# RishWijewardhena/vision-textile-inspection

Measured on AMD Instinct MI355X. Metric: frames/sec whole-node, YOLOv8n-seg 640x640 bs=64; mask IoU vs CPU ref, higher is better.
Workload: dtype f16x2

## Files before the change

vision-textile-inspection_amd/csrc/conv.hip:

```cpp
#include <algorithm>
#include <cstdlib>
#include <type_traits>

#include "conv_dev.h"

namespace vti {

__host__ __device__ inline int patch_dim(int t, int ks, int s, int mode) { return mode == 1 ? t : (t - 1) * s + ks; }

size_t stem_lds_bytes(int TH, int TW);

size_t conv_lds_bytes(int ks, int stride, int mode, int TH, int TW, int WN, int NREP) {
    if (mode == 1) return stem_lds_bytes(TH, TW);
    const int npix = patch_dim(TH, ks, stride, mode) * patch_dim(TW, ks, stride, mode);
    const size_t plane = (size_t)((npix + 15) & ~15) * 16;
    const int taps = mode == 1 ? 1 : ks * ks;
    size_t raw = 0;
    if (mode == 1) raw = (((size_t)(2 * TH + 1) * (2 * TW + 1) * 3) + 15) & ~(size_t)15;
    return 4 * plane + (size_t)WN * NREP * taps * 1024 + raw;
}

template <typename T, int KS, int S, int NREP, int WN, int NREP2 = 0, int NT = 256>
__global__ __launch_bounds__(NT, NT == 512 ? 1 : 2) void conv_kernel(const ConvParams p) {
    using vec = typename Tr<T>::vec;
    constexpr int VEC = Tr<T>::VEC, KC = Tr<T>::KC;
    constexpr int TAPS = KS * KS, PAD = KS / 2;
    constexpr int NTB = WN * NREP;
    constexpr int PP = NT / 4;
    constexpr int AR = NT == 512 ? 6 : (S == 2 ? 12 : 8);
    constexpr int BR = (NTB * TAPS * 64 + NT - 1) / NT;
    constexpr unsigned OOB = 0xFFFFFFFFu;
    extern __shared__ __attribute__((aligned(16))) char smem[];

    const int tid = threadIdx.x, lane = tid & 63, wave = tid >> 6;
    const int wn = wave % WN, wm = wave / WN;
    int t = blockIdx.x;
    const int tx = t % p.tiles_x; t /= p.tiles_x;
    const int ty = t % p.tiles_y;
    const int b = t / p.tiles_y;
    const int oy0 = ty * p.TH, ox0 = tx * p.TW;
    const int PH = (p.TH - 1) * S + KS, PW = (p.TW - 1) * S + KS;
    const int npix = PH * PW;
    const int plane_bytes = ((npix + 15) & ~15) * 16;
    char* smA = smem;
    char* smB = smem + 4 * plane_bytes;
    const int nt0 = blockIdx.y * NTB;
    const int tile_px = p.TH * p.TW;
    VTI_STAMP(0);

    int abase[MREP], opy[MREP], opx[MREP];
    bool pvalid[MREP];
#pragma unroll
    for (int m = 0; m < MREP; ++m) {
        const int pp = (wm * MREP + m) * 16 + (lane & 15);
        const bool v = pp < tile_px;
        const int pc = v ? pp : 0;
        const int py = (int)__umulhi((unsigned)pc, p.tw_magic), px = pc - py * p.TW;
        opy[m] = oy0 + py; opx[m] = ox0 + px;
        pvalid[m] = v && opy[m] < p.Hout && opx[m] < p.Wout;
        abase[m] = (lane >> 4) * plane_bytes + ((py * S) * PW + px * S) * 16;
    }

    f32x4 acc[MREP][NREP];
#pragma unroll
    for (int m = 0; m < MREP; ++m)
#pragma unroll
        for (int n = 0; n < NREP; ++n) acc[m][n] = (f32x4){0.f, 0.f, 0.f, 0.f};

    const size_t frame_elems = (size_t)p.Hin * p.Win * p.in_ld;
    const __amdgpu_buffer_rsrc_t rsA = __builtin_amdgcn_make_buffer_rsrc(
        (void*)((const T*)p.in + (size_t)b * frame_elems), 0, (int)(frame_elems * sizeof(T)), 0x00020000);
    const __amdgpu_buffer_rsrc_t rsB = __builtin_amdgcn_make_buffer_rsrc((void*)p.wpk, 0, (int)p.wpk_bytes, 0x00020000);

    const int iy0 = oy0 * S - PAD, ix0 = ox0 * S - PAD;
    const int q = (tid >> 3) & 3;
    const int pix0 = (tid >> 5) * 8 + (tid & 7);
    const int ldsA0 = q * plane_bytes + pix0 * 16;
    const int cvalid = (p.Cin - q * VEC + KC - 1) / KC;
    unsigned aoff[AR];
#pragma unroll
    for (int u = 0; u < AR; ++u) {
        const int pix = pix0 + PP * u;
        const int py = (int)__umulhi((unsigned)pix, p.pw_magic), px = pix - py * PW;
        const int y = iy0 + py, x = ix0 + px;
        const bool ok = pix < npix && (unsigned)y < (unsigned)p.Hin && (unsigned)x < (unsigned)p.Win;
        aoff[u] = ok ? (unsigned)(((y * p.Win + x) * p.in_ld + p.in_coff + q * VEC) * (int)sizeof(T)) : OOB;
    }
    constexpr bool BPRE = NREP < 5 || NT == 512;
    constexpr int PD = (KS == 1 && BPRE) ? 2 : 1;
    vec ra[PD][AR], rb[PD][BR];
    auto loadB = [&](int c, vec (&rbs)[BR]) {
        const unsigned sB = (unsigned)(((size_t)c * p.ntiles_n + nt0) * (TAPS * 1024));
#pragma unroll
        for (int u = 0; u < BR; ++u)
            if (tid + u * NT < NTB * TAPS * 64) rbs[u] = buf_load16<vec>(rsB, (unsigned)(tid + u * NT) * 16u, sB);
    };
    auto issue = [&](int c, vec (&ras)[AR], vec (&rbs)[BR]) {
        const bool qok = c < cvalid;
#pragma unroll
        for (int u = 0; u < AR; ++u)
            if (pix0 + PP * u < ((npix + 7) & ~7))
                ras[u] = buf_load16<vec>(rsA, qok ? aoff[u] : OOB, (unsigned)(c * KC * (int)sizeof(T)));
        if constexpr (BPRE) loadB(c, rbs);
    };
    auto commit = [&](int c, vec (&ras)[AR], vec (&rbs)[BR]) {
        if constexpr (!BPRE) loadB(c, rbs);
#pragma unroll
        for (int u = 0; u < AR; ++u)
            if (pix0 + PP * u < npix) *(vec*)(smA + ldsA0 + u * (PP * 16)) = ras[u];
#pragma unroll
        for (int u = 0; u < BR; ++u)
            if (tid + u * NT < NTB * TAPS * 64) *(vec*)(smB + (tid + u * NT) * 16) = rbs[u];
    };
    auto chunk = [&](int c, auto set_c) {
        constexpr int SET = decltype(set_c)::value;
        if (c < 2) VTI_STAMP(1 + 5 * c);
        commit(c, ra[SET], rb[SET]);
        if (c < 2) VTI_STAMP(3 + 5 * c);
        __syncthreads();
        if (c < 2) VTI_STAMP(4 + 5 * c);
        if (c + PD < p.nchunks) issue(c + PD, ra[SET], rb[SET]);
        {
            constexpr int NSTEP = TAPS * MREP;
            constexpr int XD = NREP >= 5 ? 2 : 3;
            constexpr int WD = NREP >= 5 ? 1 : 2;
            vec xq[XD];
            vec wq[WD][NREP];
            auto ldx = [&](int s_) -> vec {
                const int tp = s_ / MREP, mm = s_ % MREP;
                const int toff = ((tp / KS) * PW + (tp % KS)) * 16;
                return *(const vec*)(smA + abase[mm] + toff);
            };
            auto ldw = [&](int tp, vec (&w)[NREP]) {
#pragma unroll
                for (int n = 0; n < NREP; ++n)
                    w[n] = *(const vec*)(smB + ((wn * NREP + n) * TAPS + tp) * 1024 + lane * 16);
            };
            if constexpr (Tr<T>::H2 && TAPS > 1 && (NREP <= 3 || (NREP == 4 && NT == 512))) {
                auto ldw1 = [&](int tp, int n) -> vec { return *(const vec*)(smB + ((wn * NREP + n) * TAPS + tp) * 1024 + lane * 16); };
                h2_taps<NREP, MREP, TAPS, 3>(acc, ldx, ldw1);
            } else {
            ldw(0, wq[0]);
            xq[0] = ldx(0);
            if (XD > 2 && NSTEP > 1) xq[1] = ldx(1);
#pragma unroll
            for (int s_ = 0; s_ < NSTEP; ++s_) {
                const int tp = s_ / MREP, mm = s_ % MREP;
                if (s_ + XD - 1 < NSTEP) xq[(s_ + XD - 1) % XD] = ldx(s_ + XD - 1);
                if (WD == 2 && mm == 0 && tp + 1 < TAPS) ldw(tp + 1, wq[(tp + 1) % WD]);
                __builtin_amdgcn_sched_barrier(0);
#pragma unroll
                for (int n = 0; n < NREP; ++n) acc[mm][n] = mma(wq[tp % WD][n], xq[s_ % XD], acc[mm][n]);
                __builtin_amdgcn_sched_barrier(0);
                if (WD == 1 && mm == MREP - 1 && tp + 1 < TAPS) ldw(tp + 1, wq[0]);
            }
            }
        }
        if (c < 2) VTI_STAMP(5 + 5 * c);
        if (c + 1 < p.nchunks) __syncthreads();
    };

    issue(0, ra[0], rb[0]);
    if constexpr (PD == 2) {
        if (p.nchunks > 1) issue(1, ra[1], rb[1]);
        for (int c = 0; c < p.nchunks; c += 2) {
            chunk(c, std::integral_constant<int, 0>{});
            if (c + 1 < p.nchunks) chunk(c + 1, std::integral_constant<int, 1>{});
        }
    } else {
        for (int c = 0; c < p.nchunks; ++c) chunk(c, std::integral_constant<int, 0>{});
    }

    VTI_STAMP(11);
    if constexpr (NREP2 == 0) {
        conv_epilogue<T, NREP>(p, acc, pvalid, opy, opx, b, nt0, wn, lane);
    } else {
        static_assert(WN == 1, "fused stage needs the whole Cout in one wave");
        conv_stage2<T, NREP, NREP2>(p, acc, pvalid, opy, opx, b, lane);
    }
    VTI_STAMP(12);
}

size_t convfold_lds_bytes(int TH, int TW) {
    const int npix = (TH + 2) * (TW + 2);
    return 4 * (size_t)((npix + 15) & ~15) * 16 + (size_t)16 * 4 * 1024;
}
bool convfold_supported(int c_in, int c_mid, int c_out, int ntiles2) {
    return c_in == c_mid && c_mid % 16 == 0 && c_out == 64 && c_in % 16 == 0 && c_in <= 64 && combo_has(FoldN2{}, ntiles2);
}

template <typename T, int NREP2, int NT = 256>
__global__ __launch_bounds__(NT, NT == 512 ? 1 : 2) void convfold_kernel(const ConvParams p) {
    using vec = typename Tr<T>::vec;
    constexpr int VEC = Tr<T>::VEC, KC = Tr<T>::KC;
    constexpr int NREP = 4, TAPS = 4, NTB = 16, AR = 8;
    constexpr int BR = NTB * TAPS * 64 / NT;
    constexpr int PPP = NT / 4;
    constexpr unsigned OOB = 0xFFFFFFFFu;
    extern __shared__ __attribute__((aligned(16))) char smem[];

    const int tid = threadIdx.x, lane = tid & 63, wave = (tid >> 6) & 3, mgrp = tid >> 8;
    const int py = wave >> 1, px = wave & 1;
    int t = blockIdx.x;
    const int tx = t % p.tiles_x; t /= p.tiles_x;
    const int ty = t % p.tiles_y;
    const int b = t / p.tiles_y;
    const int oy0 = ty * p.TH, ox0 = tx * p.TW;
    const int PH = p.TH + 2, PW = p.TW + 2;
    const int npix = PH * PW;
    const int plane_bytes = ((npix + 15) & ~15) * 16;
    char* smA = smem;
    char* smB = smem + 4 * plane_bytes;
    const int tile_px = p.TH * p.TW;

    int abase[MREP], opy[MREP], opx[MREP];
    bool pvalid[MREP];
#pragma unroll
    for (int m = 0; m < MREP; ++m) {
        const int pp = (mgrp * MREP + m) * 16 + (lane & 15);
        const bool v = pp < tile_px;
        const int pc = v ? pp : 0;
        const int ly = (int)__umulhi((unsigned)pc, p.tw_magic), lx = pc - ly * p.TW;
        pvalid[m] = v && oy0 + ly < p.Hout && ox0 + lx < p.Wout;
        opy[m] = 2 * (oy0 + ly) + py; opx[m] = 2 * (ox0 + lx) + px;
        abase[m] = (lane >> 4) * plane_bytes + ((ly + py) * PW + lx + px) * 16;
    }
    f32x4 acc[MREP][NREP];
#pragma unroll
    for (int m = 0; m < MREP; ++m)
#pragma unroll
        for (int n = 0; n < NREP; ++n) acc[m][n] = (f32x4){0.f, 0.f, 0.f, 0.f};

    const size_t frame_elems = (size_t)p.Hin * p.Win * p.in_ld;
    const __amdgpu_buffer_rsrc_t rsA = __builtin_amdgcn_make_buffer_rsrc(
        (void*)((const T*)p.in + (size_t)b * frame_elems), 0, (int)(frame_elems * sizeof(T)), 0x00020000);
    const __amdgpu_buffer_rsrc_t rsB = __builtin_amdgcn_make_buffer_rsrc((void*)p.wpk, 0, (int)p.wpk_bytes, 0x00020000);
    const int iy0 = oy0 - 1, ix0 = ox0 - 1;
    const int q = (tid >> 3) & 3;
    const int pix0 = (tid >> 5) * 8 + (tid & 7);
    const int ldsA0 = q * plane_bytes + pix0 * 16;
    const int cvalid = (p.Cin - q * VEC + KC - 1) / KC;
    unsigned aoff[AR];
#pragma unroll
    for (int u = 0; u < AR; ++u) {
        const int pix = pix0 + PPP * u;
        const int ry = (int)__umulhi((unsigned)pix, p.pw_magic), rx = pix - ry * PW;
        const int y = iy0 + ry, x = ix0 + rx;
        const bool ok = pix < npix && (unsigned)y < (unsigned)p.Hin && (unsigned)x < (unsigned)p.Win;
        aoff[u] = ok ? (unsigned)(((y * p.Win + x) * p.in_ld + p.in_coff + q * VEC) * (int)sizeof(T)) : OOB;
    }
    vec ra[AR];
    auto issue = [&](int c) {
        const bool qok = c < cvalid;
#pragma unroll
        for (int u = 0; u < AR; ++u)
            if (pix0 + PPP * u < ((npix + 7) & ~7))
                ra[u] = buf_load16<vec>(rsA, qok ? aoff[u] : OOB, (unsigned)(c * KC * (int)sizeof(T)));
    };
    auto commit = [&](int c) {
        const unsigned sB = (unsigned)((size_t)c * (NTB * TAPS * 1024));
#pragma unroll
        for (int h = 0; h < 2; ++h) {
            vec rb[BR / 2];
#pragma unroll
            for (int u = 0; u < BR / 2; ++u) rb[u] = buf_load16<vec>(rsB, (unsigned)(tid + (h * (BR / 2) + u) * NT) * 16u, sB);
            if (h == 0) {
#pragma unroll
                for (int u = 0; u < AR; ++u)
                    if (pix0 + PPP * u < npix) *(vec*)(smA + ldsA0 + u * (PPP * 16)) = ra[u];
            }
#pragma unroll
            for (int u = 0; u < BR / 2; ++u) *(vec*)(smB + (tid + (h * (BR / 2) + u) * NT) * 16) = rb[u];
        }
    };

    issue(0);
    for (int c = 0; c < p.nchunks; ++c) {
        commit(c);
        __syncthreads();
        if (c + 1 < p.nchunks) issue(c + 1);
        {
            constexpr int NSTEP = TAPS * MREP;
            vec xq[3];
            vec wq[2][NREP];
            auto ldx = [&](int s_) -> vec {
                const int tp = s_ / MREP, mm = s_ % MREP;
                return *(const vec*)(smA + abase[mm] + ((tp >> 1) * PW + (tp & 1)) * 16);
            };
            auto ldw = [&](int tp, vec (&w)[NREP]) {
#pragma unroll
                for (int n = 0; n < NREP; ++n) w[n] = *(const vec*)(smB + ((wave * NREP + n) * TAPS + tp) * 1024 + lane * 16);
            };
            if constexpr (Tr<T>::H2) {
                auto ldw1 = [&](int tp, int n) -> vec { return *(const vec*)(smB + ((wave * NREP + n) * TAPS + tp) * 1024 + lane * 16); };
                h2_taps<NREP, MREP, TAPS, 3>(acc, ldx, ldw1);
// ... 258 lines not shown
                const int ry = wave + 4 * it;
                const int y = iy0 + ry;
                const bool row_ok = ry < SL_RH && (unsigned)y < (unsigned)p.Hin;
#pragma unroll
                for (int ch = 0; ch < RC; ++ch) {
                    const int rd = lane + 64 * ch;
                    const int gx = a0 + 4 * rd;
                    unsigned v = 0;
                    if (row_ok && rd < SL_RWD) {
#pragma unroll
                        for (int k = 0; k < 4; ++k)
                            if (gx + k >= 0 && gx + k < rowbytes) v |= (unsigned)inb[(size_t)y * rowbytes + gx + k] << (8 * k);
                    }
                    vv[it][ch] = v;
                }
            }
        }
#pragma unroll
        for (int it = 0; it < NR; ++it) {
            const int ry = wave + 4 * it;
#pragma unroll
            for (int ch = 0; ch < RC; ++ch) {
                const int rd = lane + 64 * ch;
                if (ry >= SL_RH || rd >= SL_RWD) continue;
                const unsigned v = vv[it][ch];
                PT* o = cp + (size_t)ry * SL_PITCH + 4 * rd;
                if constexpr (XH) {
                    half4 hv;
#pragma unroll
                    for (int k = 0; k < 4; ++k) hv[k] = (half_t)(float)((v >> (8 * k)) & 0xffu);
                    *(half4*)o = hv;
                } else if constexpr (sizeof(T) == 2) {
                    half4 hv;
#pragma unroll
                    for (int k = 0; k < 4; ++k) hv[k] = (half_t)((float)((v >> (8 * k)) & 0xffu) * (1.0f / 255.0f));
                    *(half4*)o = hv;
                } else {
#pragma unroll
                    for (int k = 0; k < 4; ++k) o[k] = to_T<T>((float)((v >> (8 * k)) & 0xffu) / 255.0f);
                }
            }
        }
    }
    for (int i = tid; i < SL_RH * ((SL_PITCH - 4 * SL_RWD) / 4); i += 256) {
        const int ry = i / ((SL_PITCH - 4 * SL_RWD) / 4), c4 = i - ry * ((SL_PITCH - 4 * SL_RWD) / 4);
        PT* o = cp + (size_t)ry * SL_PITCH + 4 * SL_RWD + 4 * c4;
        o[0] = to_T<PT>(0.f); o[1] = to_T<PT>(0.f); o[2] = to_T<PT>(0.f); o[3] = to_T<PT>(0.f);
    }
    __syncthreads();
    VTI_STAMP(1);
    if (aligned && t + (int)gridDim.x < ntiles) issue_raw(t + (int)gridDim.x);
    {
        const f32x4 bias4 = bias0_4;
        constexpr int NBLK = (SL_NWIN + 15) / 16;
        for (int blk = wave; blk < NBLK; blk += 4) {
            const int wi = blk * 16 + (lane & 15);
            const bool wvalid = wi < SL_NWIN;
            const int wc = wvalid ? wi : SL_NWIN - 1;
            const int J = wc / SL_SH, sy = wc - J * SL_SH;
            const PT* base = cp + (size_t)(2 * sy) * SL_PITCH + 24 * J + g * VEC;
            pvec x[3][NCH];
#pragma unroll
            for (int kh = 0; kh < 3; ++kh)
#pragma unroll
                for (int c = 0; c < NCH; ++c) x[kh][c] = *(const pvec*)(base + kh * SL_PITCH + c * KC);
            f32x4 acc[4];
#pragma unroll
            for (int pp = 0; pp < 4; ++pp) {
                acc[pp] = (f32x4){0.f, 0.f, 0.f, 0.f};
#pragma unroll
                for (int kh = 0; kh < 3; ++kh)
#pragma unroll
                    for (int c = 0; c < NCH; ++c)
#pragma unroll
                        for (int wp = 0; wp < NWP; ++wp) acc[pp] = mma(wA[pp][kh][c * NWP + wp], x[kh][c], acc[pp]);
            }
            const bool row_in = (unsigned)(sy0 + sy) < (unsigned)Hs;
#pragma unroll
            for (int pp = 0; pp < 4; ++pp) {
                const int sx = 4 * J + pp;
                f32x4 v = silu4<FAST>(acc_bias<T>(acc[pp], bias4, p.alpha0));
                if (!(row_in && (unsigned)(sx0 + sx) < (unsigned)Ws)) v = (f32x4){0.f, 0.f, 0.f, 0.f};
                if (wvalid && sx < SL_SW) {
                    T* o = (T*)(sout + ((size_t)(sy * SL_SW + sx) * 16 + g * 4) * ES);
                    if constexpr (sizeof(T) == 2) {
                        half4 hv;
#pragma unroll
                        for (int j = 0; j < 4; ++j) hv[j] = (half_t)v[j];
                        *(half4*)o = hv;
                    } else {
                        *(u32x4*)o = pack4<T>(v);
                    }
                }
            }
        }
    }
    __syncthreads();
    VTI_STAMP(2);
    int opy[MREP], opx[MREP], sbase[MREP];
    bool pvalid[MREP];
#pragma unroll
    for (int m = 0; m < MREP; ++m) {
        const int pp = (wave * MREP + m) * 16 + (lane & 15);
        const int py = pp / SL_TW, px = pp - py * SL_TW;
        opy[m] = oy0 + py; opx[m] = ox0 + px;
        pvalid[m] = opy[m] < p.Hout && opx[m] < p.Wout;
        sbase[m] = ((2 * py) * SL_SW + 2 * px) * 16 * ES;
    }
    f32x4 acc[MREP][2];
#pragma unroll
    for (int m = 0; m < MREP; ++m) { acc[m][0] = (f32x4){0.f, 0.f, 0.f, 0.f}; acc[m][1] = (f32x4){0.f, 0.f, 0.f, 0.f}; }
#pragma unroll
    for (int s = 0; s < NS1; ++s) {
        const int tap = sizeof(T) == 2 ? 2 * s + (g >> 1) : s;
        const int tc = tap < 9 ? tap : 8;
        const int toff = ((tc / 3) * SL_SW + (tc % 3)) * 16 * ES + (sizeof(T) == 2 ? (g & 1) * 8 : g * 4) * ES;
        vec w1[2];
#pragma unroll
        for (int n = 0; n < 2; ++n) w1[n] = w1all[s][n];
#pragma unroll
        for (int m = 0; m < MREP; ++m) {
            const vec x = *(const vec*)(sout + sbase[m] + toff);
#pragma unroll
            for (int n = 0; n < 2; ++n) acc[m][n] = mma(w1[n], x, acc[m][n]);
        }
    }
    VTI_STAMP(3);
    if (p.out2) conv_stage2<T, 2, 2, false, true>(p, acc, pvalid, opy, opx, b, lane, &s2r);
    else conv_epilogue<T, 2>(p, acc, pvalid, opy, opx, b, 0, 0, lane);
    VTI_STAMP(12);
    }
}

void stem_l1_tile(int* th, int* tw) { *th = SL_TH; *tw = SL_TW; }

int stem_l1_grid(int dtype, int ntiles) {
    const int wgpc = (int)std::min<size_t>(2, (160 * 1024) / stem_l1_lds_bytes(dtype));
    const char* np = getenv("VTI_STEM_NOT_PERSISTENT");
    if (np && np[0] == '1') return ntiles;
    return std::min(ntiles, 256 * std::max(1, wgpc));
}

hipError_t launch_stem_l1(int dtype, const ConvParams& p, hipStream_t st) {
    dim3 grid((unsigned)stem_l1_grid(dtype, p.B * p.tiles_y * p.tiles_x));
    if (grid.x == 0) return hipSuccess;
    const size_t lds = stem_l1_lds_bytes(dtype);
    return with_conv_type(dtype, [&](auto t) { return launch_lds<stem_l1_kernel<typename decltype(t)::type>>(grid, dim3(256), lds, st, p); });
}

size_t stem_lds_bytes(int TH, int TW) { return 1024 + (size_t)(2 * TH + 1) * ((((2 * TW + 1) * 3 + 6) >> 2) * 4); }

using ConvTile3 = Combos<Ints<1, 1>, Ints<2, 1>, Ints<3, 1>, Ints<4, 1>, Ints<5, 1>, Ints<1, 2>, Ints<2, 2>, Ints<1, 4>>;
using ConvTile1 = decltype(concat(ConvTile3{}, Combos<Ints<3, 2>, Ints<4, 2>, Ints<5, 2>, Ints<2, 4>, Ints<3, 4>, Ints<4, 4>, Ints<5, 4>>{}));
using StemNrep = Combos<Ints<1>, Ints<2>, Ints<3>, Ints<4>, Ints<5>>;

bool conv_cfg_fits(int ks, int stride, int mode, int TH, int TW, int WN, int NREP, int threads) {
    if (mode == 1) return WN == 1 && (2 * TH + 1) * (((2 * TW + 1) * 3 + 6) >> 2) < 65536;
    if (threads != 256 && !(threads == 512 && ks == 3 && stride == 1 && WN == 1)) return false;
    const int AR = threads == 512 ? 6 : (stride == 2 ? 12 : 8);
    const int npix = patch_dim(TH, ks, stride, mode) * patch_dim(TW, ks, stride, mode);
    if (((npix + 7) / 8) * 32 > threads * AR) return false;
    return ks == 1 ? combo_has(ConvTile1{}, NREP, WN) : combo_has(ConvTile3{}, NREP, WN);
}

bool conv_fusable(int nrep, int nrep2) { return combo_has(FusedPairs{}, nrep, nrep2); }

template <typename T, int KS, int S>
static hipError_t launch_ks(int nrep, const ConvParams& p, dim3 grid, size_t lds, hipStream_t st) {
    return combo_dispatch(std::conditional_t<KS == 1, ConvTile1, ConvTile3>{}, [&](auto c) {
        using C = decltype(c);
        return launch_lds<conv_kernel<T, KS, S, C::v[0], C::v[1]>>(grid, dim3(256), lds, st, p);
    }, nrep, p.WN);
}

template <typename T>
static hipError_t launch_t(int ks, int stride, int nrep, int mode, const ConvParams& p, dim3 grid, size_t lds,
                           hipStream_t st) {
    if (p.ntiles2 > 0) {
        if (!(ks == 3 && stride == 1 && p.WN == 1 && mode == 0)) return hipErrorInvalidValue;
        return combo_dispatch(FusedPairs{}, [&](auto c) {
            using C = decltype(c);
            return p.nt == 512 ? launch_lds<conv_kernel<T, 3, 1, C::v[0], 1, C::v[1], 512>>(grid, dim3(512), lds, st, p)
                               : launch_lds<conv_kernel<T, 3, 1, C::v[0], 1, C::v[1]>>(grid, dim3(256), lds, st, p);
        }, nrep, p.ntiles2);
    }
    if (mode == 1)
        return combo_dispatch(StemNrep{}, [&](auto c) {
            hipLaunchKernelGGL((stem_kernel<T, decltype(c)::v[0]>), grid, dim3(256), lds, st, p);
            return hipGetLastError();
        }, nrep);
    if (ks == 1 && stride == 1) return launch_ks<T, 1, 1>(nrep, p, grid, lds, st);
    if (ks == 3 && stride == 1) return launch_ks<T, 3, 1>(nrep, p, grid, lds, st);
    if (ks == 3 && stride == 2) return launch_ks<T, 3, 2>(nrep, p, grid, lds, st);
    return hipErrorInvalidValue;
}

hipError_t launch_conv(int dtype, int ks, int stride, int nrep, int mode, const ConvParams& p, size_t lds_bytes,
                       hipStream_t st) {
    if (p.pk == 4) return launch_conv_pk2(dtype, nrep, p, lds_bytes, st);
    if (p.pk == 3) return launch_bneck_pk(dtype, nrep, p, lds_bytes, st);
    if (p.pk == 2) return launch_conv1_pk(dtype, nrep, p, lds_bytes, st);
    if (p.pk) return launch_conv_pk(dtype, nrep, p, lds_bytes, st);
    const int NTB = p.WN * nrep;
    dim3 grid((unsigned)(p.B * p.tiles_y * p.tiles_x), (unsigned)((p.ntiles_n + NTB - 1) / NTB));
    if (grid.x == 0) return hipSuccess;
    const int nwaves = p.nt == 512 ? 8 : 4;
    if ((p.nt != 256 && p.nt != 512) || (p.nt == 512 && p.ntiles2 == 0)) return hipErrorInvalidValue;
    if (p.TH * p.TW > (nwaves / p.WN) * MREP * 16 || (p.WN != 1 && p.WN != 2 && p.WN != 4)) return hipErrorInvalidValue;
    return with_conv_type(dtype, [&](auto t) { return launch_t<typename decltype(t)::type>(ks, stride, nrep, mode, p, grid, lds_bytes, st); });
}

}
```

vision-textile-inspection_amd/csrc/conv_pk.hip:

```cpp
#include <algorithm>
#include <cstdlib>
#include <type_traits>

#include "conv_dev.h"

namespace vti {

constexpr int PK_PWP = 24;
constexpr int PK_TW = 20;
constexpr int PK_ROWS = 4;
constexpr int PK_MAXD = 9;
constexpr int PK_MAXD2 = 13;

using ConvPkS1 = Combos<Ints<1, 1>, Ints<2, 1>, Ints<3, 1>, Ints<4, 1>, Ints<5, 1>, Ints<1, 2>, Ints<2, 2>, Ints<3, 2>, Ints<4, 2>, Ints<1, 4>,
                        Ints<2, 4>>;
using ConvPkS2 = Combos<Ints<1, 4>, Ints<2, 2>, Ints<4, 1>, Ints<2, 1>, Ints<1, 2>>;
using Conv1Pk = decltype(concat(ConvPkS1{}, Combos<Ints<4, 4>>{}));
bool conv_pk_instantiated(int nrep, int wn) { return combo_has(ConvPkS1{}, nrep, wn); }
bool conv_pk2_instantiated(int nrep, int wn) { return combo_has(ConvPkS2{}, nrep, wn); }
bool conv1_pk_instantiated(int nrep, int wn) { return combo_has(Conv1Pk{}, nrep, wn); }

static size_t pk_stage_bytes(int TH, int S) { return S == 2 ? (size_t)(2 * TH + 1) * 2 * PK_PWP * 64 : (size_t)(TH + 2) * PK_PWP * 64; }
size_t conv_pk2_lds_bytes(int TH, int WN, int NREP, int nchunks, int depth, int wstat) {
    const int nwbuf = wstat ? nchunks : nchunks > 2 ? depth : (nchunks > 1 ? 2 : 1);
    return depth * pk_stage_bytes(TH, 2) + (size_t)nwbuf * WN * NREP * 9 * 1024 + (size_t)WN * NREP * 16 * 4;
}
bool conv_pk2_fits(int TH, int WN, int NREP, int nchunks, int wstat) {
    if (TH % PK_ROWS || !conv_pk2_instantiated(NREP, WN)) return false;
    const int ncomp = (TH / PK_ROWS) * WN;
    if (ncomp < 1 || ncomp > 4) return false;
    const int ndma = (int)(pk_stage_bytes(TH, 2) / 1024);
    if ((ndma + ncomp - 1) / ncomp > PK_MAXD2) return false;
    return conv_pk2_lds_bytes(TH, WN, NREP, nchunks, 2, wstat) <= 160 * 1024;
}
int conv_pk2_depth(int TH, int WN, int NREP, int nchunks, int wstat) {
    if (!conv_pk2_fits(TH, WN, NREP, nchunks, wstat)) return 0;
    const char* cap = getenv("VTI_PK_DEPTH");
    const int maxd = cap ? std::max(2, std::min(4, atoi(cap))) : 2;
    const int ncomp = (TH / PK_ROWS) * WN;
    const int per_step = ((int)(pk_stage_bytes(TH, 2) / 1024) + ncomp - 1) / ncomp + (nchunks > 2 && !wstat ? (WN * NREP * 9 + ncomp - 1) / ncomp : 0);
    int d = 2;
    while (d < maxd && conv_pk2_lds_bytes(TH, WN, NREP, nchunks, d + 1, wstat) <= 160 * 1024 && per_step * (d - 1) <= 63) ++d;
    return d;
}

size_t conv_pk_lds_bytes(int TH, int WN, int NREP, int nchunks, int depth, int wstat) {
    const size_t stage = (size_t)(TH + 2) * PK_PWP * 64;
    const int nwbuf = wstat ? nchunks : nchunks > 2 ? depth : (nchunks > 1 ? 2 : 1);
    return depth * stage + (size_t)nwbuf * WN * NREP * 9 * 1024 + (size_t)WN * NREP * 16 * 4;
}
size_t conv_pk_lds_bytes(int TH, int WN, int NREP, int nchunks) { return conv_pk_lds_bytes(TH, WN, NREP, nchunks, 2, 0); }

int conv_pk_depth(int TH, int WN, int NREP, int nchunks, int wstat) {
    if (!conv_pk_fits(TH, WN, NREP, nchunks, wstat)) return 0;
    const char* cap = getenv("VTI_PK_DEPTH");
    const int maxd = cap ? std::max(2, std::min(4, atoi(cap))) : 2;
    const int ncomp = (TH / PK_ROWS) * WN;
    const int per_step = ((TH + 2) * PK_PWP / 16 + ncomp - 1) / ncomp + (nchunks > 2 && !wstat ? (WN * NREP * 9 + ncomp - 1) / ncomp : 0);
    int d = 2;
    while (d < maxd && conv_pk_lds_bytes(TH, WN, NREP, nchunks, d + 1, wstat) <= 160 * 1024 && per_step * (d - 1) <= 63) ++d;
    return d;
}

bool conv_pk_fits(int TH, int WN, int NREP, int nchunks, int wstat) {
    if (TH % PK_ROWS) return false;
    const int ncomp = (TH / PK_ROWS) * WN;
    if (ncomp < 1 || ncomp > 4) return false;
    const int ndma = (TH + 2) * PK_PWP / 16;
    if ((ndma + ncomp - 1) / ncomp > PK_MAXD) return false;
    return conv_pk_lds_bytes(TH, WN, NREP, nchunks, 2, wstat) <= 160 * 1024;
}

__device__ __forceinline__ void dma16(__amdgpu_buffer_rsrc_t r, unsigned voff, unsigned soff, unsigned lds_addr) {
    unsigned keep;
    asm volatile("s_mov_b32 %0, m0\n\ts_mov_b32 m0, %1\n\ts_nop 0\n\tbuffer_load_dwordx4 %2, %3, %4 offen lds\n\ts_mov_b32 m0, %0"
                 : "=&s"(keep) : "s"(lds_addr), "v"(voff), "s"(r), "s"(soff) : "memory");
}

template <int N> __device__ __forceinline__ void wait_vm() { asm volatile("s_waitcnt vmcnt(%0)" :: "i"(N) : "memory"); }
template <int N> struct WaitVm { static __device__ __forceinline__ void go(int n) { if (n >= N) wait_vm<N>(); else WaitVm<N - 1>::go(n); } };
template <> struct WaitVm<0> { static __device__ __forceinline__ void go(int) { wait_vm<0>(); } };

__device__ __forceinline__ void pk_stagger_wait(int units) {
    if (units > 0 && (int)(blockIdx.x >> 3) * 2 >= (int)(gridDim.x >> 3))
        for (int i = 0; i < units; ++i) __builtin_amdgcn_s_sleep(16);
}

template <typename T, int NREP, int WN, int NREP2 = 0, bool FOLD = false, int S = 1>
__global__ __launch_bounds__(512) void conv3_pk(const ConvParams p) {
    using vec = typename Tr<T>::vec;
    constexpr int VEC = Tr<T>::VEC, KC = Tr<T>::KC, ES = (int)sizeof(T);
    constexpr int TAPS = FOLD ? 4 : 9, NTB = WN * NREP;
    constexpr int PWP = S == 2 ? 2 * PK_PWP : PK_PWP;
    constexpr int MAXD = S == 2 ? PK_MAXD2 : PK_MAXD;
    static_assert(S == 1 || (S == 2 && !FOLD && NREP2 == 0), "stride 2: plain epilogue only");
    constexpr int WCHUNK = NTB * TAPS * 1024;
    constexpr unsigned OOB = 0x80000000u;
    constexpr bool FAST = !Tr<T>::F32;
    extern __shared__ __attribute__((aligned(16))) char smem[];

    const int tid = threadIdx.x, lane = tid & 63;
    const int wave = __builtin_amdgcn_readfirstlane(tid >> 6);
    static_assert(!FOLD || (WN == 4 && NREP2 > 0), "fold: one compute wave per output phase, fused 1x1 epilogue");
    const int ncomp = (p.TH / PK_ROWS) * WN;
    const int nld = (int)(blockDim.x >> 6) - ncomp;
    const int PH = S == 2 ? 2 * p.TH + 1 : p.TH + 2;
    const int stage_bytes = PH * PWP * 64;
    const int ndma = PH * PWP / 16;
    const int D = p.pk_depth;
    const bool stream_w = p.nchunks > 2 && !p.pk_wstat;
    const int wbuf_off = D * stage_bytes;
    const int bias_off = wbuf_off + (stream_w ? D : p.nchunks) * WCHUNK;
    const unsigned lds0 = (unsigned)(size_t)(__attribute__((address_space(3))) char*)smem;
    const int nt0 = blockIdx.y * NTB;

    for (int i = tid; i < NTB * 16; i += (int)blockDim.x) ((float*)(smem + bias_off))[i] = p.bias[nt0 * 16 + i];
    __syncthreads();

    int t, tend, tstride;
    if (p.pk_xcd) {
        const int per = (p.pk_tiles + 7) >> 3, k = blockIdx.x & 7;
        t = k * per + (int)(blockIdx.x >> 3);
        tend = min((k + 1) * per, p.pk_tiles);
        tstride = (int)(gridDim.x >> 3);
    } else {
        t = blockIdx.x; tend = p.pk_tiles; tstride = (int)gridDim.x;
    }
    if (t >= tend) return;
    auto tile_coords = [&](int tt, int& b, int& oy0, int& ox0) {
        const int tx = tt % p.tiles_x, r = tt / p.tiles_x;
        const int ty = r % p.tiles_y;
        b = r / p.tiles_y; oy0 = ty * p.TH; ox0 = tx * PK_TW;
    };
    const int nsteps = ((tend - t + tstride - 1) / tstride) * p.nchunks;

    if (wave >= ncomp) {
        const int lw = wave - ncomp;
        const int q = (lane & 3) ^ (((lane >> 4) & 1) << 1);
        const int cvalid = (p.Cin - q * VEC + KC - 1) / KC;
        int dyx[MAXD];
#pragma unroll
        for (int u = 0; u < MAXD; ++u) {
            const int s = (lw + u * nld) * 16 + (lane >> 2);
            if constexpr (S == 2) {
                const int py = (int)(((unsigned)s * 1366u) >> 16), r = s - py * PWP;
                const int plane = r >= PK_PWP ? 1 : 0, idx = r - plane * PK_PWP;
                dyx[u] = idx < PK_TW + 1 - plane ? (py << 8) | (2 * idx + plane) : -1;
            } else {
                const int py = (int)(((unsigned)s * 2731u) >> 16), px = s - py * PK_PWP;
                dyx[u] = px < PK_TW + 2 ? (py << 8) | px : -1;
            }
        }
        const __amdgpu_buffer_rsrc_t rsA = __builtin_amdgcn_make_buffer_rsrc((void*)p.in, 0, (int)p.in_bytes, 0x00020000);
        const __amdgpu_buffer_rsrc_t rsB = __builtin_amdgcn_make_buffer_rsrc((void*)p.wpk, 0, (int)p.wpk_bytes, 0x00020000);
        unsigned voff[MAXD];
        auto setup_voff = [&](int tt) {
            int b, oy0, ox0;
            tile_coords(tt, b, oy0, ox0);
#pragma unroll
            for (int u = 0; u < MAXD; ++u) {
                const int y = S * oy0 - 1 + (dyx[u] >> 8), x = S * ox0 - 1 + (dyx[u] & 255);
                const bool ok = dyx[u] >= 0 && (unsigned)y < (unsigned)p.Hin && (unsigned)x < (unsigned)p.Win;
                voff[u] = ok ? (unsigned)((((b * p.Hin + y) * p.Win + x) * p.in_ld + p.in_coff + q * VEC) * ES) : OOB;
            }
        };
        auto issue_patch = [&](int c, int stage) {
            const bool qok = c < cvalid;
            const unsigned dst = lds0 + stage * stage_bytes + lw * 1024;
#pragma unroll
            for (int u = 0; u < MAXD; ++u)
                if (lw + u * nld < ndma)
                    dma16(rsA, qok ? voff[u] : OOB, (unsigned)(c * KC * ES), dst + u * nld * 1024);
        };
// ... 83 lines not shown
                vec wq[WD][NREP];
                auto ldx = [&](int s_) -> vec {
                    const int tp = s_ / MREP, mm = s_ % MREP;
                    if constexpr (FOLD) return *(const vec*)(sx + xa[mm][tp & 1] + (tp >> 1) * (PK_PWP * 64));
                    else return *(const vec*)(sx + xa[mm][tp % 3] + (tp / 3) * (PWP * 64));
                };
                auto ldw = [&](int tp, vec (&w)[NREP]) {
#pragma unroll
                    for (int n = 0; n < NREP; ++n) w[n] = *(const vec*)(sw + (n * TAPS + tp) * 1024);
                };
                if constexpr (Tr<T>::H2) {
                    auto ldw1 = [&](int tp, int n) -> vec { return *(const vec*)(sw + (n * TAPS + tp) * 1024); };
#ifndef H2_XD
#define H2_XD (NREP >= 4 ? 3 : 4)
#endif
                    if constexpr (NREP >= 5) h2_taps_nmajor<NREP, MREP, TAPS>(acc, ldx, ldw1);
                    else h2_taps<NREP, MREP, TAPS, H2_XD>(acc, ldx, ldw1);
                } else {
                ldw(0, wq[0]);
#pragma unroll
                for (int i = 0; i < XD - 1; ++i) xq[i] = ldx(i);
#pragma unroll
                for (int s_ = 0; s_ < NSTEP; ++s_) {
                    const int tp = s_ / MREP, mm = s_ % MREP;
                    if (s_ + XD - 1 < NSTEP) xq[(s_ + XD - 1) % XD] = ldx(s_ + XD - 1);
                    if (mm == 0 && tp + 1 < TAPS) ldw(tp + 1, wq[(tp + 1) % WD]);
                    __builtin_amdgcn_sched_barrier(0);
#pragma unroll
                    for (int n = 0; n < NREP; ++n) acc[mm][n] = mma(wq[tp % WD][n], xq[s_ % XD], acc[mm][n]);
                    __builtin_amdgcn_sched_barrier(0);
                }
                }
            }
            if (step < 2) VTI_STAMP(3 + 4 * step);
        }
        VTI_STAMP(11);
        if (fast_epi) {
            const int crun = (nt0 + wn * NREP) * 16 + (lane >> 4) * 4 * NREP;
            const char* sb = smem + bias_off + (wn * NREP * 16 + (lane >> 4) * 4 * NREP) * 4;
            f32x4 bias_r[NREP];
#pragma unroll
            for (int n = 0; n < NREP; ++n) bias_r[n] = *(const f32x4*)(sb + n * 16);
            auto epi = [&](auto has_res_c) {
            constexpr bool has_res = decltype(has_res_c)::value;
            constexpr bool RES_UPFRONT = has_res && sizeof(T) == 2 && NREP <= 2;
            typedef unsigned u32x2 __attribute__((ext_vector_type(2)));
            u32x2 rr[RES_UPFRONT ? MREP : 1][RES_UPFRONT ? NREP : 1];
            if constexpr (RES_UPFRONT) {
#pragma unroll
                for (int m = 0; m < MREP; ++m) {
                    const int gy = oy0 + ry[m], gx = ox0 + rx[m];
                    const bool pv = gy < p.Hout && gx < p.Wout;
                    const int opix = (b * p.Hout + gy) * p.Wout + gx;
                    const unsigned rb = (unsigned)((opix * p.res_ld + p.res_coff + crun) * ES);
#pragma unroll
                    for (int n = 0; n < NREP; ++n)
                        rr[m][n] = __builtin_amdgcn_raw_buffer_load_b64(rsR, (pv && crun + 4 * n < p.Cout) ? rb + n * 8 : OOB, 0u, 0);
                }
            }
#pragma unroll
            for (int m = 0; m < MREP; ++m) {
                const int gy = oy0 + ry[m], gx = ox0 + rx[m];
                const bool pv = gy < p.Hout && gx < p.Wout;
                const int opix = (b * p.Hout + gy) * p.Wout + gx;
                const unsigned ob = (unsigned)((opix * p.out_ld + p.out_coff + crun) * ES);
                f32x4 v[NREP];
                if constexpr (RES_UPFRONT) {
#pragma unroll
                    for (int n = 0; n < NREP; ++n) {
                        const half4 r = __builtin_bit_cast(half4, rr[m][n]);
#pragma unroll
                        for (int j = 0; j < 4; ++j) v[n][j] = (float)r[j];
                    }
                } else if constexpr (has_res) {
                    const unsigned rb = (unsigned)((opix * p.res_ld + p.res_coff + crun) * ES);
#pragma unroll
                    for (int n = 0; n < NREP; ++n) {
                        const bool cv = pv && crun + 4 * n < p.Cout;
                        if constexpr (sizeof(T) == 2) {
                            const u32x2 r2 = __builtin_amdgcn_raw_buffer_load_b64(rsR, cv ? rb + n * 8 : OOB, 0u, 0);
                            const half4 r = __builtin_bit_cast(half4, r2);
#pragma unroll
                            for (int j = 0; j < 4; ++j) v[n][j] = (float)r[j];
                        } else {
                            v[n] = unpack4<T>(buf_load16<u32x4>(rsR, cv ? rb + n * 16 : OOB, 0u));
                        }
                    }
                }
#pragma unroll
                for (int n = 0; n < NREP; ++n) {
                    f32x4 a = acc_bias<T>(acc[m][n], bias_r[n], p.alpha);
                    if (p.act) a = silu4<FAST>(a);
                    if constexpr (has_res) v[n] += a; else v[n] = a;
                }
                if constexpr (sizeof(T) == 2 && NREP % 2 == 0) {
#pragma unroll
                    for (int n = 0; n < NREP; n += 2) {
                        half8 hv;
#pragma unroll
                        for (int j = 0; j < 4; ++j) { hv[j] = (half_t)v[n][j]; hv[4 + j] = (half_t)v[n + 1][j]; }
                        const bool cv = pv && crun + 4 * n + 8 <= p.Cout;
                        __builtin_amdgcn_raw_buffer_store_b128(__builtin_bit_cast(u32x4, hv), rsO, cv ? ob + n * 8 : OOB, 0u, 0);
                    }
                } else if constexpr (sizeof(T) == 2) {
                    typedef unsigned u32x2 __attribute__((ext_vector_type(2)));
#pragma unroll
                    for (int n = 0; n < NREP; ++n) {
                        half4 hv;
#pragma unroll
                        for (int j = 0; j < 4; ++j) hv[j] = (half_t)v[n][j];
                        const bool cv = pv && crun + 4 * n < p.Cout;
                        __builtin_amdgcn_raw_buffer_store_b64(__builtin_bit_cast(u32x2, hv), rsO, cv ? ob + n * 8 : OOB, 0u, 0);
                    }
                } else {
#pragma unroll
                    for (int n = 0; n < NREP; ++n) {
                        const bool cv = pv && crun + 4 * n < p.Cout;
                        __builtin_amdgcn_raw_buffer_store_b128(pack4<T>(v[n]), rsO, cv ? ob + n * 16 : OOB, 0u, 0);
                    }
                }
            }
            };
            if (p.has_res) epi(std::true_type{}); else epi(std::false_type{});
        } else {
            int opy[MREP], opx[MREP];
            bool pvalid[MREP];
#pragma unroll
            for (int m = 0; m < MREP; ++m) {
                opy[m] = oy0 + ry[m]; opx[m] = ox0 + rx[m];
                pvalid[m] = opy[m] < p.Hout && opx[m] < p.Wout;
            }
            if constexpr (FOLD) {
#pragma unroll
                for (int m = 0; m < MREP; ++m) { opy[m] = 2 * opy[m] + fpy; opx[m] = 2 * opx[m] + fpx; }
                const bool interior = oy0 > 0 && oy0 + p.TH < p.Hout && ox0 > 0 && ox0 + PK_TW < p.Wout;
                conv_stage2<T, NREP, NREP2, true, true>(p, acc, pvalid, opy, opx, b, lane, &s2r, interior);
            } else if constexpr (NREP2 == 0) conv_epilogue<T, NREP>(p, acc, pvalid, opy, opx, b, nt0, wn, lane);
            else conv_stage2<T, NREP, NREP2>(p, acc, pvalid, opy, opx, b, lane);
        }
        VTI_STAMP(12);
        const int tn = t + tstride;
        if (tn >= tend) break;
        t = tn;
        tile_coords(t, b, oy0, ox0);
    }
}


constexpr int PK1_MAXP = 5;

size_t conv1_pk_lds_bytes(int nwm, int WN, int NREP, int nchunks, int depth, int wstat, int cps) {
    const size_t stage = (size_t)nwm * 80 * 64 * cps;
    const size_t wch = (size_t)WN * NREP * 1024;
    return (size_t)depth * stage + (wstat ? (size_t)nchunks * wch : (size_t)depth * wch * cps) + 1024  + (size_t)WN * NREP * 64;
}

template <typename T, int NREP, int WN, int CPS>
__global__ __launch_bounds__(512) void conv1_pk(const ConvParams p) {
    using vec = typename Tr<T>::vec;
    constexpr int VEC = Tr<T>::VEC, KC = Tr<T>::KC, ES = (int)sizeof(T);
    constexpr int NTB = WN * NREP;
    constexpr int WCH = NTB * 1024;
    constexpr unsigned OOB = 0x80000000u;
    constexpr bool FAST = !Tr<T>::F32;
    extern __shared__ __attribute__((aligned(16))) char smem[];

    const int tid = threadIdx.x, lane = tid & 63;
    const int wave = __builtin_amdgcn_readfirstlane(tid >> 6);
    const int nwm = p.TH;
    const int ncomp = nwm * WN;
    const int nld = (int)(blockDim.x >> 6) - ncomp;
    const int D = p.pk_depth;
    const int tile_px = nwm * 80;
    const int img_bytes = tile_px * 64;
    const int stage_bytes = img_bytes * CPS;
    const int npieces = tile_px / 16;
    const int wbuf_off = D * stage_bytes;
    const int dummy_off = wbuf_off + (p.pk_wstat ? p.nchunks : D * CPS) * WCH;
    const int spt = (p.nchunks + CPS - 1) / CPS;
    const int bias_off = dummy_off + 1024;
    const unsigned lds0 = (unsigned)(size_t)(__attribute__((address_space(3))) char*)smem;
    const int nt0 = blockIdx.y * NTB;
    const int total_px = p.B * p.Hout * p.Wout;

    for (int i = tid; i < NTB * 16; i += (int)blockDim.x) ((float*)(smem + bias_off))[i] = p.bias[nt0 * 16 + i];
    __syncthreads();

    int t, tend, tstride;
    if (p.pk_xcd) {
        const int per = (p.pk_tiles + 7) >> 3, k = blockIdx.x & 7;
        t = k * per + (int)(blockIdx.x >> 3);
        tend = min((k + 1) * per, p.pk_tiles);
        tstride = (int)(gridDim.x >> 3);
    } else {
        t = blockIdx.x; tend = p.pk_tiles; tstride = (int)gridDim.x;
    }
    if (t >= tend) return;
    const int ntiles_mine = (tend - t + tstride - 1) / tstride;
    const int nsteps = ntiles_mine * spt;

    if (wave >= ncomp) {
        const int lw = wave - ncomp;
        const int q = (lane & 3) ^ (((lane >> 4) & 1) << 1);
        const int cvalid = (p.Cin - q * VEC + KC - 1) / KC;
        const __amdgpu_buffer_rsrc_t rsA = __builtin_amdgcn_make_buffer_rsrc((void*)p.in, 0, (int)p.in_bytes, 0x00020000);
        const __amdgpu_buffer_rsrc_t rsB = __builtin_amdgcn_make_buffer_rsrc((void*)p.wpk, 0, (int)p.wpk_bytes, 0x00020000);
        const int ppl = (npieces + nld - 1) / nld;
        const int wpl = p.pk_wstat ? 0 : (NTB + nld - 1) / nld;
        const int per_step = CPS * (ppl + wpl);
        const __amdgpu_buffer_rsrc_t rsA2 = __builtin_amdgcn_make_buffer_rsrc((void*)p.in2, 0, (int)p.in2_bytes, 0x00020000);
        unsigned vo1[PK1_MAXP], vo2[PK1_MAXP];
        int cur_ti = -1;
        auto issue = [&](int s) {
            const int ti = s / spt, cs = s - ti * spt;
            if (ti != cur_ti) {
                cur_ti = ti;
                const int pix0 = (t + ti * tstride) * tile_px;
                const int hw = p.Hout * p.Wout;
#pragma unroll
                for (int u = 0; u < PK1_MAXP; ++u) {
                    const int piece = lw + u * nld;
                    const int px = pix0 + piece * 16 + (lane >> 2);
                    const bool ok = piece < npieces && px < total_px;
                    vo1[u] = ok ? (unsigned)((px * p.in_ld + p.in_coff + q * VEC) * ES) : OOB;
                    vo2[u] = OOB;
                    if (p.up_C > 0 && ok) {
                        const int bb = px / hw, r = px - bb * hw;
                        const int y = r / p.Wout, x = r - y * p.Wout;
                        const int px2 = (bb * (p.Hout >> 1) + (y >> 1)) * (p.Wout >> 1) + (x >> 1);
                        vo2[u] = (unsigned)((px2 * p.in2_ld + p.in2_coff + q * VEC) * ES);
                    }
                }
            }
            const int slot = s % D;
#pragma unroll
            for (int cc = 0; cc < CPS; ++cc) {
                const int c = cs * CPS + cc;
                const bool live = c < p.nchunks;
                const bool qok = c < cvalid && live;
                const bool from_up = c * KC < p.up_C;
                const unsigned dst = lds0 + slot * stage_bytes + cc * img_bytes;
#pragma unroll
                for (int u = 0; u < PK1_MAXP; ++u) {
                    if (u >= ppl) break;
                    const int piece = lw + u * nld;
                    const unsigned vo = qok ? (from_up ? vo2[u] : vo1[u]) : OOB;
                    const unsigned ld = piece < npieces ? dst + piece * 1024 : lds0 + dummy_off;
                    if (from_up) dma16(rsA2, vo, (unsigned)(c * KC * ES), ld);
                    else dma16(rsA, vo, (unsigned)(c * KC * ES), ld);
                }
                if (wpl) {
                    const unsigned src = (unsigned)(((size_t)(live ? c : 0) * p.ntiles_n + nt0) * 1024);
                    const unsigned wd = lds0 + wbuf_off + (slot * CPS + cc) * WCH;
                    for (int u = 0; u < wpl; ++u) {
                        const int f = lw + u * nld;
                        dma16(rsB, (f < NTB && live) ? (unsigned)lane * 16u : OOB, src + f * 1024, f < NTB ? wd + f * 1024 : lds0 + dummy_off);
                    }
                }
            }
        };
        if (p.pk_wstat) {
            for (int f = lw; f < p.nchunks * NTB; f += nld) {
                const int c = f / NTB, n = f - c * NTB;
                dma16(rsB, (unsigned)lane * 16u, (unsigned)(((size_t)c * p.ntiles_n + nt0 + n) * 1024), lds0 + wbuf_off + f * 1024);
            }
        }
        const int ahead = min(D - 1, nsteps);
        for (int s = 0; s < ahead; ++s) issue(s);
        for (int s = 0; s < nsteps; ++s) {
            const int inflight = min(D - 2, nsteps - 1 - s);
            WaitVm<63>::go(min(63, inflight * per_step));
            __builtin_amdgcn_s_barrier();
            if (s + D - 1 < nsteps) issue(s + D - 1);
        }
        return;
    }

    const int wn = wave % WN, wm = wave / WN;
    int xa[MREP];
#pragma unroll
    for (int m = 0; m < MREP; ++m) {
        const int sl = wm * 80 + m * 16 + (lane & 15);
        xa[m] = (sl * 64 + (lane >> 4) * 16) ^ ((sl & 4) << 3);
    }
    const __amdgpu_buffer_rsrc_t rsO = __builtin_amdgcn_make_buffer_rsrc(p.out, 0, (int)p.out_bytes, 0x00020000);
    const bool fast_epi = !p.scalar_store && !p.out_f32 && !p.deconv_c && !p.has_res &&
                          (sizeof(T) != 2 || NREP % 2 || (p.Cout & 7) == 0);
    const int crun = (nt0 + wn * NREP) * 16 + (lane >> 4) * 4 * NREP;
    int s = 0;
    for (int ti = 0; ti < ntiles_mine; ++ti) {
        f32x4 acc[MREP][NREP];
#pragma unroll
        for (int m = 0; m < MREP; ++m)
#pragma unroll
            for (int n = 0; n < NREP; ++n) acc[m][n] = (f32x4){0.f, 0.f, 0.f, 0.f};
        for (int cs = 0; cs < spt; ++cs, ++s) {
            __builtin_amdgcn_s_barrier();
            asm volatile("" ::: "memory");
            const int slot = s % D;
            const int ncc = min(CPS, p.nchunks - cs * CPS);
            if constexpr (Tr<T>::H2) {
                constexpr int NU = CPS * NREP;
                const int nu = ncc * NREP;
                auto wptr = [&](int u) -> const char* {
                    const int cc = u / NREP, n = u - cc * NREP;
                    return smem + wbuf_off + (p.pk_wstat ? cs * CPS + cc : slot * CPS + cc) * WCH + (wn * NREP + n) * 1024 + lane * 16;
                };
                u32x4 wraw[2], wh[2], wl[2];
                h2x4 x[2][MREP];
                wraw[0] = *(const u32x4*)wptr(0);
                if (nu > 1) wraw[1] = *(const u32x4*)wptr(1);
#pragma unroll
                for (int m = 0; m < MREP; ++m) x[0][m] = *(const h2x4*)(smem + slot * stage_bytes + xa[m]);
#pragma unroll
                for (int i = 0; i < 4; ++i) { wh[0][i] = __builtin_amdgcn_perm(wraw[0][i], wraw[0][i], 0x01000100u); wl[0][i] = wraw[0][i] >> 16; }
#pragma unroll
                for (int u = 0; u < NU; ++u) {
                    if (u < nu) {
                        const int cc = u / NREP, n = u % NREP, cur = u & 1, nxt = cur ^ 1;
                        if (n == 0 && cc + 1 < CPS && cc + 1 < ncc) {
#pragma unroll
                            for (int m = 0; m < MREP; ++m) x[(cc + 1) & 1][m] = *(const h2x4*)(smem + slot * stage_bytes + (cc + 1) * img_bytes + xa[m]);
                        }
                        u32x4 wnext = wraw[nxt];
                        if (u + 2 < nu) wraw[cur] = *(const u32x4*)wptr(u + 2);
                        __builtin_amdgcn_sched_barrier(0);
#pragma unroll
                        for (int j = 0; j < 2 * MREP; ++j) {
                            const int m = j >> 1;
                            acc[m][n] = __builtin_amdgcn_mfma_f32_16x16x32_f16(__builtin_bit_cast(half8, (j & 1) ? wl[cur] : wh[cur]),
                                                                               __builtin_bit_cast(half8, x[cc & 1][m].u), acc[m][n], 0, 0, 0);
                            if (j < 8 && u + 1 < nu) {
                                const int i = j & 3;
                                if (j < 4) wh[nxt][i] = __builtin_amdgcn_perm(wnext[i], wnext[i], 0x01000100u);
                                else wl[nxt][i] = wnext[i] >> 16;
                                __builtin_amdgcn_sched_group_barrier(0x008, 1, 0);
                                __builtin_amdgcn_sched_group_barrier(0x002, 1, 0);
                            }
                        }
                        __builtin_amdgcn_sched_barrier(0);
                    }
                }
            } else {
#pragma unroll
                for (int cc = 0; cc < CPS; ++cc) {
                    if (cc < ncc) {
                        const int c = cs * CPS + cc;
                        const char* sx = smem + slot * stage_bytes + cc * img_bytes;
                        const char* sw = smem + wbuf_off + (p.pk_wstat ? c : slot * CPS + cc) * WCH + wn * (NREP * 1024) + lane * 16;
                        vec w[NREP];
#pragma unroll
                        for (int n = 0; n < NREP; ++n) w[n] = *(const vec*)(sw + n * 1024);
                        vec x[MREP];
#pragma unroll
                        for (int m = 0; m < MREP; ++m) x[m] = *(const vec*)(sx + xa[m]);
#pragma unroll
                        for (int m = 0; m < MREP; ++m)
#pragma unroll
                            for (int n = 0; n < NREP; ++n) acc[m][n] = mma(w[n], x[m], acc[m][n]);
                    }
                }
            }
        }
        const int pix0 = (t + ti * tstride) * tile_px + wm * 80;
        if (fast_epi) {
            const char* sb = smem + bias_off + (wn * NREP * 16 + (lane >> 4) * 4 * NREP) * 4;
            f32x4 bias_r[NREP];
#pragma unroll
            for (int n = 0; n < NREP; ++n) bias_r[n] = *(const f32x4*)(sb + n * 16);
#pragma unroll
            for (int m = 0; m < MREP; ++m) {
                const int opix = pix0 + m * 16 + (lane & 15);
                const bool pv = opix < total_px;
                const unsigned ob = (unsigned)((opix * p.out_ld + p.out_coff + crun) * ES);
                f32x4 v[NREP];
#pragma unroll
                for (int n = 0; n < NREP; ++n) {
                    v[n] = acc_bias<T>(acc[m][n], bias_r[n], p.alpha);
                    if (p.act) v[n] = silu4<FAST>(v[n]);
                }
                if constexpr (sizeof(T) == 2 && NREP % 2 == 0) {
#pragma unroll
                    for (int n = 0; n < NREP; n += 2) {
                        half8 hv;
#pragma unroll
                        for (int j = 0; j < 4; ++j) { hv[j] = (half_t)v[n][j]; hv[4 + j] = (half_t)v[n + 1][j]; }
                        const bool cv = pv && crun + 4 * n + 8 <= p.Cout;
                        __builtin_amdgcn_raw_buffer_store_b128(__builtin_bit_cast(u32x4, hv), rsO, cv ? ob + n * 8 : OOB, 0u, 0);
                    }
                } else if constexpr (sizeof(T) == 2) {
                    typedef unsigned u32x2 __attribute__((ext_vector_type(2)));
#pragma unroll
                    for (int n = 0; n < NREP; ++n) {
                        half4 hv;
#pragma unroll
                        for (int j = 0; j < 4; ++j) hv[j] = (half_t)v[n][j];
                        const bool cv = pv && crun + 4 * n < p.Cout;
                        __builtin_amdgcn_raw_buffer_store_b64(__builtin_bit_cast(u32x2, hv), rsO, cv ? ob + n * 8 : OOB, 0u, 0);
                    }
                } else {
#pragma unroll
                    for (int n = 0; n < NREP; ++n) {
                        const bool cv = pv && crun + 4 * n < p.Cout;
                        __builtin_amdgcn_raw_buffer_store_b128(pack4<T>(v[n]), rsO, cv ? ob + n * 16 : OOB, 0u, 0);
                    }
                }
            }
        } else {
            int opy[MREP], opx[MREP];
            bool pvalid[MREP];
            const int hw = p.Hout * p.Wout;
            int bfr = 0;
#pragma unroll
            for (int m = 0; m < MREP; ++m) {
                const int opix = pix0 + m * 16 + (lane & 15);
                pvalid[m] = opix < total_px;
                const int oc = pvalid[m] ? opix : 0;
                const int bb = oc / hw, r = oc - bb * hw;
                opy[m] = r / p.Wout; opx[m] = r - opy[m] * p.Wout;
                opy[m] += bb * p.Hout;
            }
            conv_epilogue<T, NREP>(p, acc, pvalid, opy, opx, bfr, nt0, wn, lane);
        }
    }
}

bool conv1_pk_fits(int nwm, int WN, int NREP, int nchunks, int depth, int wstat, int cps) {
    const int ncomp = nwm * WN;
    if (nwm < 1 || ncomp > 4 || depth < 2 || depth > 8 || cps < 1 || cps > 2) return false;
    const int npieces = nwm * 5;
    if ((npieces + ncomp - 1) / ncomp > PK1_MAXP) return false;
    const int per_step = cps * ((npieces + ncomp - 1) / ncomp + (wstat ? 0 : (WN * NREP + ncomp - 1) / ncomp));
    if (per_step * (depth - 2) > 63) return false;
    return conv1_pk_lds_bytes(nwm, WN, NREP, nchunks, depth, wstat, cps) <= 160 * 1024;
}

hipError_t launch_conv1_pk(int dtype, int nrep, const ConvParams& p, size_t lds_bytes, hipStream_t st) {
    const int NTB = p.WN * nrep;
    if (!conv1_pk_fits(p.TH, p.WN, nrep, p.nchunks, p.pk_depth, p.pk_wstat, p.pk_cps)) return hipErrorInvalidValue;
    if (p.ntiles_n % NTB || p.pk_wgs < 1 || (p.pk_xcd && p.pk_wgs % 8) || p.has_res) return hipErrorInvalidValue;
    if ((size_t)p.in_bytes >= 0x80000000u || (size_t)p.out_bytes >= 0x80000000u) return hipErrorInvalidValue;
    if (p.pk_tiles == 0) return hipSuccess;
    const int threads = 2 * p.TH * p.WN * 64;
    dim3 grid((unsigned)p.pk_wgs, (unsigned)(p.ntiles_n / NTB));
    return with_conv_type(dtype, [&](auto t) {
        using T = typename decltype(t)::type;
        constexpr int CPS = sizeof(T) == 2 ? 1 : 2;
        if (p.pk_cps != CPS) return hipErrorInvalidValue;
        return combo_dispatch(Conv1Pk{}, [&](auto c) {
            using C = decltype(c);
            return launch_lds<conv1_pk<T, C::v[0], C::v[1], CPS>>(grid, dim3(threads), lds_bytes, st, p);
        }, nrep, p.WN);
    });
}

size_t conv_pk_fold_lds_bytes(int nchunks, int depth) { return depth * (size_t)6 * PK_PWP * 64 + (size_t)(nchunks > 1 ? 2 : 1) * 16 * 4 * 1024 + 16 * 16 * 4; }
int conv_pk_fold_depth(int nchunks) {
    const char* cap = getenv("VTI_PK_FOLD_DEPTH");
    const int maxd = cap ? std::max(2, std::min(4, atoi(cap))) : 3;
    int d = 2;
    while (d < maxd && conv_pk_fold_lds_bytes(nchunks, d + 1) <= 160 * 1024) ++d;
    return d;
}

hipError_t launch_conv_pk_fold(int dtype, const ConvParams& p, size_t lds_bytes, hipStream_t st) {
    if (p.TH != 4 || p.TW != PK_TW || p.WN != 4 || p.nchunks > 2 || p.ntiles_n != 16 || !p.fold || !p.out2) return hipErrorInvalidValue;
    if (p.pk_wgs < 1 || (p.pk_xcd && p.pk_wgs % 8) || (size_t)p.in_bytes >= 0x80000000u) return hipErrorInvalidValue;
    if (p.pk_depth < 2 || p.pk_depth > 4 || lds_bytes < conv_pk_fold_lds_bytes(p.nchunks, p.pk_depth) || lds_bytes > 160 * 1024) return hipErrorInvalidValue;
    if (p.pk_tiles == 0) return hipSuccess;
    dim3 grid((unsigned)p.pk_wgs, 1);
    return combo_dispatch(FoldN2{}, [&](auto c) {
        return with_conv_type(dtype, [&](auto t) {
            return launch_lds<conv3_pk<typename decltype(t)::type, 4, 4, decltype(c)::v[0], true>>(grid, dim3(512), lds_bytes, st, p);
        });
    }, p.ntiles2);
}

hipError_t launch_conv_pk2(int dtype, int nrep, const ConvParams& p, size_t lds_bytes, hipStream_t st) {
    const int NTB = p.WN * nrep;
    if (p.TW != PK_TW || !conv_pk2_fits(p.TH, p.WN, nrep, p.nchunks, p.pk_wstat) || p.ntiles2 > 0) return hipErrorInvalidValue;
    if (p.pk_depth < 2 || p.pk_depth > 4 || lds_bytes < conv_pk2_lds_bytes(p.TH, p.WN, nrep, p.nchunks, p.pk_depth, p.pk_wstat) || lds_bytes > 160 * 1024) return hipErrorInvalidValue;
    if (p.ntiles_n % NTB || p.pk_wgs < 1 || (p.pk_xcd && p.pk_wgs % 8)) return hipErrorInvalidValue;
    if ((size_t)p.in_bytes >= 0x80000000u || (size_t)p.out_bytes >= 0x80000000u) return hipErrorInvalidValue;
    if (p.pk_tiles == 0) return hipSuccess;
    const int threads = 2 * (p.TH / PK_ROWS) * p.WN * 64;
    dim3 grid((unsigned)p.pk_wgs, (unsigned)(p.ntiles_n / NTB));
    return combo_dispatch(ConvPkS2{}, [&](auto c) {
        return with_conv_type(dtype, [&](auto t) {
            using C = decltype(c);
            return launch_lds<conv3_pk<typename decltype(t)::type, C::v[0], C::v[1], 0, false, 2>>(grid, dim3(threads), lds_bytes, st, p);
        });
    }, nrep, p.WN);
}

hipError_t launch_conv_pk(int dtype, int nrep, const ConvParams& p, size_t lds_bytes, hipStream_t st) {
    const int NTB = p.WN * nrep;
    if (p.TH % PK_ROWS || p.TW != PK_TW || !conv_pk_fits(p.TH, p.WN, nrep, p.nchunks, p.pk_wstat)) return hipErrorInvalidValue;
    if (p.pk_depth < 2 || p.pk_depth > 4 || lds_bytes < conv_pk_lds_bytes(p.TH, p.WN, nrep, p.nchunks, p.pk_depth, p.pk_wstat) || lds_bytes > 160 * 1024) return hipErrorInvalidValue;
    if (p.ntiles_n % NTB || p.pk_wgs < 1 || (p.pk_xcd && p.pk_wgs % 8)) return hipErrorInvalidValue;
    if ((size_t)p.in_bytes >= 0x80000000u || (size_t)p.out_bytes >= 0x80000000u) return hipErrorInvalidValue;
    if (p.pk_tiles == 0) return hipSuccess;
    const int threads = 2 * (p.TH / PK_ROWS) * p.WN * 64;
    dim3 grid((unsigned)p.pk_wgs, (unsigned)(p.ntiles_n / NTB));
    return with_conv_type(dtype, [&](auto t) {
        using T = typename decltype(t)::type;
        if (p.ntiles2 > 0) {
            if (p.WN != 1) return hipErrorInvalidValue;
            return combo_dispatch(FusedPairs{}, [&](auto c) {
                using C = decltype(c);
                return launch_lds<conv3_pk<T, C::v[0], 1, C::v[1]>>(grid, dim3(threads), lds_bytes, st, p);
            }, nrep, p.ntiles2);
        }
        return combo_dispatch(ConvPkS1{}, [&](auto c) {
            using C = decltype(c);
            return launch_lds<conv3_pk<T, C::v[0], C::v[1]>>(grid, dim3(threads), lds_bytes, st, p);
        }, nrep, p.WN);
    });
}

constexpr int BN_MREP1 = 7;

size_t bneck_pk_lds_bytes(int TH, int NREP, int depth) {
    return depth * (size_t)(TH + 4) * PK_PWP * 64 + (size_t)(TH + 2) * PK_PWP * 64 + 2 * (size_t)NREP * 9 * 1024 + 2 * (size_t)NREP * 64;
}
size_t bneck_pk_lds_bytes(int TH, int NREP) { return bneck_pk_lds_bytes(TH, NREP, 2); }
int bneck_pk_depth(int TH, int NREP) {
    const char* cap = getenv("VTI_PK_DEPTH");
    const int maxd = cap ? std::max(2, std::min(4, atoi(cap))) : 2;
    const int nwm = TH / PK_ROWS;
    const int per_step = ((TH + 4) * PK_PWP / 16 + nwm - 1) / nwm;
    int d = 2;
    while (d < maxd && bneck_pk_lds_bytes(TH, NREP, d + 1) <= 160 * 1024 && per_step * (d - 1) <= 63) ++d;
    return d;
}
bool bneck_pk_fits(int TH, int NREP) {
    if (TH % PK_ROWS || TH < 8 || TH > 16 || NREP < 1 || NREP > 2) return false;
    const int nwm = TH / PK_ROWS;
    if (((TH + 2) * (PK_TW + 2) + 15) / 16 > BN_MREP1 * nwm) return false;
    if (((TH + 4) * PK_PWP / 16 + nwm - 1) / nwm > PK_MAXD) return false;
    return bneck_pk_lds_bytes(TH, NREP) <= 160 * 1024;
}

template <typename T, int NREP, bool TAIL = false>
__global__ __launch_bounds__(512) void bneck_pk(const ConvParams p) {
    static_assert(!TAIL || ((sizeof(T) == 2 || Tr<T>::H2) && NREP == 1), "tail: fp16 / h2, 16 channels");
    constexpr bool TAILH2 = TAIL && Tr<T>::H2;
    using vec = typename Tr<T>::vec;
    constexpr int VEC = Tr<T>::VEC, ES = (int)sizeof(T);
    constexpr int TAPS = 9, R1W = PK_TW + 2;
    constexpr unsigned OOB = 0x80000000u;
    constexpr bool FAST = !Tr<T>::F32;
    extern __shared__ __attribute__((aligned(16))) char smem[];

    const int tid = threadIdx.x, lane = tid & 63, g = lane >> 4;
    const int wave = __builtin_amdgcn_readfirstlane(tid >> 6);
    const int nwm = p.TH / PK_ROWS;
    const int PH = p.TH + 4, R1H = p.TH + 2;
    const int stage_bytes = PH * PK_PWP * 64;
    const int D = p.pk_depth;
    const int timg_off = D * stage_bytes;
    const int w1_off = timg_off + R1H * PK_PWP * 64;
    const int w2_off = w1_off + NREP * TAPS * 1024;
    const int bias_off = w2_off + NREP * TAPS * 1024;
    const unsigned lds0 = (unsigned)(size_t)(__attribute__((address_space(3))) char*)smem;

    for (int i = tid; i < NREP * 16; i += (int)blockDim.x) {
        ((float*)(smem + bias_off))[i] = p.bias[i];
        ((float*)(smem + bias_off))[NREP * 16 + i] = p.bias2[i];
    }
    for (int i = tid; i < R1H * PK_PWP * 4; i += (int)blockDim.x) ((f32x4*)(smem + timg_off))[i] = (f32x4){0.f, 0.f, 0.f, 0.f};
    __syncthreads();

    int t, tend, tstride;
    if (p.pk_xcd) {
        const int per = (p.pk_tiles + 7) >> 3, k = blockIdx.x & 7;
        t = k * per + (int)(blockIdx.x >> 3);
        tend = min((k + 1) * per, p.pk_tiles);
        tstride = (int)(gridDim.x >> 3);
    } else {
        t = blockIdx.x; tend = p.pk_tiles; tstride = (int)gridDim.x;
    }
    if (t >= tend) return;
    auto tile_coords = [&](int tt, int& b, int& oy0, int& ox0) {
        const int tx = tt % p.tiles_x, r = tt / p.tiles_x;
        const int ty = r % p.tiles_y;
        b = r / p.tiles_y; oy0 = ty * p.TH; ox0 = tx * PK_TW;
    };
    const int ntiles_mine = (tend - t + tstride - 1) / tstride;

    if (wave >= nwm) {
        const int lw = wave - nwm, nld = nwm;
        const int ndma = PH * PK_PWP / 16;
        const int q = (lane & 3) ^ (((lane >> 4) & 1) << 1);
        const bool qok = q * VEC < ((TAIL && !TAILH2) ? 2 * p.Cin : p.Cin);
        int dyx[PK_MAXD];
#pragma unroll
        for (int u = 0; u < PK_MAXD; ++u) {
            const int s = (lw + u * nld) * 16 + (lane >> 2);
            const int py = (int)(((unsigned)s * 2731u) >> 16), px = s - py * PK_PWP;
            dyx[u] = (py << 8) | px;
        }
// ... 355 lines not shown
```

vision-textile-inspection_amd/csrc/plan.cpp:

```cpp
#include <algorithm>
#include <cmath>
#include <cstdio>
#include <cstdlib>
#include <cstring>

#include "vti_internal.h"

namespace vti {

namespace {

struct Scale { char tag; double depth, width; int maxc; };
const Scale kScales[] = {{'n', 0.33, 0.25, 1024}, {'s', 0.33, 0.50, 1024}, {'m', 0.67, 0.75, 768},
                         {'l', 1.00, 1.00, 512},  {'x', 1.00, 1.25, 512}};

int make_divisible(double x, int d) { return (int)std::ceil(x / d) * d; }
int py_round(double x) { return (int)std::nearbyint(x); }

struct Builder {
    Plan& P;
    int maxB;
    std::vector<Op>* cur;
    int lane = 0;
    explicit Builder(Plan& p) : P(p), maxB(p.desc.max_batch), cur(&p.ops) {}
// ... 32 lines not shown
        const Buf& ib = P.bufs[in.buf];
        const int c = out.C / 2;
        const int Y = new_buf((2 + n) * c, ib.H, ib.W);
        char nm[64];
        snprintf(nm, sizeof nm, "model.%d.cv1", idx);
        conv(nm, in, slice(Y, 0, 2 * c), 1, 1, 0);
        for (int j = 0; j < n; ++j) {
            const int T = new_buf(c, ib.H, ib.W);
            View prev = slice(Y, (1 + j) * c, c);
            snprintf(nm, sizeof nm, "model.%d.m.%d.cv1", idx, j);
            conv(nm, prev, whole(T), 3, 1, 0);
            snprintf(nm, sizeof nm, "model.%d.m.%d.cv2", idx, j);
            conv(nm, whole(T), slice(Y, (2 + j) * c, c), 3, 1, 0, false, shortcut ? &prev : nullptr);
        }
        snprintf(nm, sizeof nm, "model.%d.cv2", idx);
        conv(nm, whole(Y), out, 1, 1, 0);
    }

    void up2(View in, View out) {
        Op op; op.kind = OP_UP2; op.in = in; op.out = out; op.lane = lane;
        cur->push_back(op);
    }
};

}

static bool choose_pk_cfg(int dtype, const ConvRow& r, int max_batch, ConvCfg& c, int fth, int fwn, int fnrep) {
    const char* no = getenv("VTI_NO_PK");
    if (no && no[0] == '1') return false;
    if (!(r.k == 3 && r.s == 1 && r.kind != 2) || r.w_out < 20) return false;
    const int esize = dtype == VTI_F16 ? 2 : 4;
    static const bool wide16 = getenv("VTI_PK_WIDE16") && getenv("VTI_PK_WIDE16")[0] == '1';
    const bool wide = dtype != VTI_F16 || wide16;
    const double mf = dtype == VTI_H2 ? 2.0 : dtype == VTI_F32 ? 8.0 : 1.0;
    static const bool no_wstat = getenv("VTI_NO_PK_WSTAT") && getenv("VTI_NO_PK_WSTAT")[0] == '1';
    double best = 1e30;
    bool found = false;
    const int tiles_x = (r.w_out + 19) / 20;
    for (int WN = 1; WN <= 4; WN *= 2) {
        if (fwn && WN != fwn) continue;
        for (int NREP = 1; NREP <= 5; ++NREP) {
            if (fnrep && NREP != fnrep) continue;
            if (!conv_pk_instantiated(NREP, WN)) continue;
            static const bool h2_no_n5 = getenv("VTI_H2_NO_N5") && getenv("VTI_H2_NO_N5")[0] == '1';
            if (dtype == VTI_H2 && NREP == 5 && !fnrep && h2_no_n5) continue;
            const int NTB = WN * NREP;
            const int gy = (c.ntiles_n + NTB - 1) / NTB;
            const double n_eff = (double)c.ntiles_n / (gy * NTB);
            if (n_eff < 0.74 && !fnrep) continue;
            for (int NWM = 1; NWM <= 4; ++NWM) {
                const int TH = 4 * NWM, ncomp = NWM * WN;
                if (fth && TH != fth) continue;
                for (int wstat = (wide && !no_wstat && c.nchunks > 2) ? 1 : 0; wstat >= 0; --wstat) {
                    if (ncomp > 4 || !conv_pk_fits(TH, WN, NREP, c.nchunks, wstat)) continue;
                    const size_t lds = conv_pk_lds_bytes(TH, WN, NREP, c.nchunks, 2, wstat);
                    const int wgpc = (int)std::min<size_t>(2, (160 * 1024) / lds);
                    const int tiles_y = (r.h_out + TH - 1) / TH;
                    const long NT = (long)max_batch * tiles_y * tiles_x;
                    const long G = pk_grid(NT, wgpc, gy);
                    const long rounds = (NT + G - 1) / G;
                    const int simd_load = (ncomp * wgpc + 3) / 4;
                    const double lds_reads = (1.0 / NREP + 0.2) / mf;
                    const double solo = wide ? ((ncomp * wgpc > 4) ? 1.1 : 1.45) : 1.0;
                    const double mfma_cyc = (double)c.nchunks * 45 * NREP * 16 * mf * solo * std::max(1.0, lds_reads / 0.5) * (NREP == 5 ? 1.6 : 1.0);
                    const double t_comp = rounds * (mfma_cyc * simd_load + 1100.0 * NREP) / 1.9e9;
                    const double bytes = (double)NT * ((double)gy * (TH + 2) * 22 * r.c1 + (double)TH * 20 * r.c2) * esize;
                    const double t_mem = bytes / 5.0e12;
                    double t_ing = 0.0;
                    if (wide) {
                        const double patch = (double)(TH + 2) * 24 * 64 * c.nchunks, wbytes = (double)NTB * 9 * 1024 * c.nchunks;
                        const bool resident = wstat || c.nchunks <= 2;
                        t_ing = ((double)NT * gy * (patch + (resident ? 0.0 : wbytes)) + (resident ? (double)G * gy * wbytes : 0.0)) / 8.0e12;
                    }
                    const double cost = (std::max(std::max(t_comp, t_mem), t_ing) + 0.15 * std::min(t_comp, t_mem)) * (wide ? 1.0 + 0.06 * (gy - 1) : 1.0) + 4e-6;
                    if (cost < best) {
                        best = cost; found = true;
                        c.TH = TH; c.TW = 20; c.WN = WN; c.NREP = NREP; c.lds = lds; c.pk = 1; c.pk_wgpc = wgpc; c.pk_wstat = wstat;
                    }
                }
            }
        }
    }
    if (found) {
        c.ntiles_n = (c.ntiles_n + c.WN * c.NREP - 1) / (c.WN * c.NREP) * (c.WN * c.NREP);
        c.pk_depth = 2;
        const int dmax = conv_pk_depth(c.TH, c.WN, c.NREP, c.nchunks, c.pk_wstat);
        for (int dd = 3; dd <= dmax; ++dd) {
            const size_t l = conv_pk_lds_bytes(c.TH, c.WN, c.NREP, c.nchunks, dd, c.pk_wstat);
            if ((int)std::min<size_t>(2, (160 * 1024) / l) >= c.pk_wgpc) { c.pk_depth = dd; c.lds = l; }
        }
    }
    return found;
}

static bool choose_pk2_cfg(int dtype, const ConvRow& r, int max_batch, ConvCfg& c, int fth, int fwn, int fnrep) {
    const char* no = getenv("VTI_NO_PK2");
    if (no && no[0] == '1') return false;
    if (!(r.k == 3 && r.s == 2 && r.kind == 0) || r.w_out < 20) return false;
    const int esize = dtype == VTI_F16 ? 2 : 4;
    static const bool wide16 = getenv("VTI_PK_WIDE16") && getenv("VTI_PK_WIDE16")[0] == '1';
    const bool wide = dtype != VTI_F16 || wide16;
    const double mf = dtype == VTI_H2 ? 2.0 : dtype == VTI_F32 ? 8.0 : 1.0;
    static const bool no_wstat = getenv("VTI_NO_PK_WSTAT") && getenv("VTI_NO_PK_WSTAT")[0] == '1';
    double best = 1e30;
    bool found = false;
    const int tiles_x = (r.w_out + 19) / 20;
    for (int WN = 1; WN <= 4; WN *= 2) {
        if (fwn && WN != fwn) continue;
        for (int NREP = 1; NREP <= 4; ++NREP) {
            if (fnrep && NREP != fnrep) continue;
            if (!conv_pk2_instantiated(NREP, WN)) continue;
            const int NTB = WN * NREP;
            const int gy = (c.ntiles_n + NTB - 1) / NTB;
            const double n_eff = (double)c.ntiles_n / (gy * NTB);
            if (n_eff < 0.74 && !fnrep) continue;
            for (int NWM = 1; NWM <= 4; ++NWM) {
                const int TH = 4 * NWM, ncomp = NWM * WN;
                if (fth && TH != fth) continue;
                for (int wstat = (wide && !no_wstat && c.nchunks > 2) ? 1 : 0; wstat >= 0; --wstat) {
                    if (ncomp > 4 || !conv_pk2_fits(TH, WN, NREP, c.nchunks, wstat)) continue;
                    const int tiles_y = (r.h_out + TH - 1) / TH;
                    const long NT = (long)max_batch * tiles_y * tiles_x;
                    const long G = pk_grid(NT, 1, gy);
                    const long rounds = (NT + G - 1) / G;
                    const int simd_load = (ncomp + 3) / 4;
                    const double lds_reads = (1.0 / NREP + 0.2) / mf;
                    const double mfma_cyc = (double)c.nchunks * 45 * NREP * 16 * mf * std::max(1.0, lds_reads / 0.5);
                    const double t_comp = rounds * (mfma_cyc * simd_load + 1100.0 * NREP) / 1.9e9;
                    const double bytes = (double)NT * ((double)gy * (2 * TH + 1) * 41 * r.c1 + (double)TH * 20 * r.c2) * esize;
                    const double t_mem = bytes / 5.0e12;
                    double t_ing = 0.0;
                    if (wide) {
                        const double patch = (double)(2 * TH + 1) * 48 * 64 * c.nchunks, wbytes = (double)NTB * 9 * 1024 * c.nchunks;
                        const bool resident = wstat || c.nchunks <= 2;
                        t_ing = ((double)NT * gy * (patch + (resident ? 0.0 : wbytes)) + (resident ? (double)G * gy * wbytes : 0.0)) / 8.0e12;
                    }
                    const double cost = std::max(std::max(t_comp, t_mem), t_ing) + 0.15 * std::min(t_comp, t_mem) + 4e-6;
                    if (cost < best) {
                        best = cost; found = true;
                        c.TH = TH; c.TW = 20; c.WN = WN; c.NREP = NREP; c.pk = 4; c.pk_wgpc = 1; c.pk_wstat = wstat;
                    }
                }
            }
        }
    }
    if (found) {
        c.ntiles_n = (c.ntiles_n + c.WN * c.NREP - 1) / (c.WN * c.NREP) * (c.WN * c.NREP);
        c.pk_depth = conv_pk2_depth(c.TH, c.WN, c.NREP, c.nchunks, c.pk_wstat);
        c.lds = conv_pk2_lds_bytes(c.TH, c.WN, c.NREP, c.nchunks, c.pk_depth, c.pk_wstat);
    }
    return found;
}

static bool choose_pk1_cfg(int esize, const ConvRow& r, int max_batch, ConvCfg& c, int fth, int fwn, int fnrep) {
    const int cps = esize == 2 ? 1 : 2;
    const char* no = getenv("VTI_NO_PK1");
    if (no && no[0] == '1') return false;
    const bool deconv = r.kind == 2;
    if (!((r.k == 1 && r.s == 1) || deconv)) return false;
    const bool forced = fth || fwn || fnrep;
    const char* all1 = getenv("VTI_PK1_ALL");
    if (!forced && !(all1 && all1[0] == '1') && (deconv || r.h_out * r.w_out < 1600)) return false;
    const long total_px = (long)max_batch * (deconv ? r.h_in * r.w_in : r.h_out * r.w_out);
    double best = 1e30;
    bool found = false;
    for (int WN = 1; WN <= 4; WN *= 2) {
        if (fwn && WN != fwn) continue;
        for (int NREP = 1; NREP <= 5; ++NREP) {
            if (fnrep && NREP != fnrep) continue;
            if (!conv1_pk_instantiated(NREP, WN)) continue;
            if (deconv && r.c2 % (16 * NREP)) continue;
            const int NTB = WN * NREP;
            const int gy = (c.ntiles_n + NTB - 1) / NTB;
            const double n_eff = (double)c.ntiles_n / (gy * NTB);
            if (n_eff < 0.74 && !fnrep) continue;
            for (int nwm = 1; nwm <= 4; ++nwm) {
                if (fth && nwm != fth) continue;
                const int ncomp = nwm * WN;
                if (ncomp > 4) continue;
                static const size_t wstat_max = getenv("VTI_PK1_WSTAT_KB") ? (size_t)atoi(getenv("VTI_PK1_WSTAT_KB")) * 1024 : 96 * 1024;
                const int wstat = (size_t)c.nchunks * NTB * 1024 <= wstat_max ? 1 : 0;
                static const bool no_w2 = getenv("VTI_PK1_NO_WGPC2") && getenv("VTI_PK1_NO_WGPC2")[0] == '1';
                static const bool force_w2 = getenv("VTI_PK1_FORCE_WGPC2") && getenv("VTI_PK1_FORCE_WGPC2")[0] == '1';
                for (int wgpc = (esize == 4 && force_w2) ? 2 : 1; wgpc <= ((esize == 4 && !no_w2) ? 2 : 1); ++wgpc) {
                    int depth = 0;
                    for (int dd = 8; dd >= 2; --dd)
                        if (conv1_pk_fits(nwm, WN, NREP, c.nchunks, dd, wstat, cps) &&
                            conv1_pk_lds_bytes(nwm, WN, NREP, c.nchunks, dd, wstat, cps) <= (size_t)(160 * 1024) / wgpc) { depth = dd; break; }
                    if (!depth) continue;
                    const long NT = (total_px + nwm * 80 - 1) / (nwm * 80);
                    const long G = pk_grid(NT, wgpc, gy);
                    const long rounds = (NT + G - 1) / G;
                    const double solo = esize == 4 ? ((ncomp * wgpc > 4) ? 1.1 : 1.45) : 1.0;
                    const double step_cyc = 5.0 * NREP * 16 * solo * (esize == 4 ? 2.0 : 1.0) + 250.0 / cps;
                    const double t_comp = rounds * (c.nchunks * step_cyc + 1100.0 * NREP) * ((ncomp * wgpc + 3) / 4) / 1.9e9;
                    const double bytes = (double)total_px * ((double)gy * r.c1 + (double)c.gemm_n) * esize +
                                         (wstat ? 0.0 : (double)NT * gy * c.nchunks * NTB * 1024 * 0.25);
                    const double inflight = (double)wgpc * (depth - 1) * nwm * 80 * 64 * cps;
                    static const double inflight_full = getenv("VTI_PK1_INFLIGHT_KB") ? atof(getenv("VTI_PK1_INFLIGHT_KB")) * 1e3 : 50e3;
                    const double t_mem = bytes / (5.0e12 * std::min(1.0, inflight / inflight_full));
                    const double cost = std::max(t_comp, t_mem) + 0.15 * std::min(t_comp, t_mem) + 4e-6;
                    if (cost < best) {
                        best = cost; found = true;
                        c.TH = nwm; c.TW = 80; c.WN = WN; c.NREP = NREP; c.pk = 2; c.pk_wgpc = wgpc; c.pk_depth = depth; c.pk_wstat = wstat; c.pk_cps = cps;
                        c.lds = conv1_pk_lds_bytes(nwm, WN, NREP, c.nchunks, depth, wstat, cps);
                    }
                }
            }
        }
    }
    if (found) c.ntiles_n = (c.ntiles_n + c.WN * c.NREP - 1) / (c.WN * c.NREP) * (c.WN * c.NREP);
    return found;
}

void choose_conv_cfg(int dtype, const ConvRow& r, bool conv0, int max_batch, ConvCfg& c, int fth, int ftw, int fwn,
                     int fnrep, bool allow_pk) {
    const bool f16 = dtype == VTI_F16;
    const int KC = f16 ? 32 : 16;
    const bool deconv = r.kind == 2;
    c.gemm_n = deconv ? 4 * r.c2 : r.c2;
    c.ntiles_n = (c.gemm_n + 15) / 16;
    c.nchunks = conv0 ? (32 / KC) : (r.c1 + KC - 1) / KC;
    c.pk = 0;
    if (allow_pk && !conv0 && (!ftw || ftw == 80) && (!fth || fth <= 4) && choose_pk1_cfg(f16 ? 2 : 4, r, max_batch, c, fth, fwn, fnrep)) return;
    c.pk_wstat = 0;
    if (allow_pk && !conv0 && (!ftw || ftw == 20) && (!fth || fth % 4 == 0) && choose_pk_cfg(dtype, r, max_batch, c, fth, fwn, fnrep)) {
        return;
    }
    if (allow_pk && !conv0 && (!ftw || ftw == 20) && (!fth || fth % 4 == 0) && choose_pk2_cfg(dtype, r, max_batch, c, fth, fwn, fnrep)) return;
    const int ks = deconv ? 1 : r.k, st = deconv ? 1 : r.s;
    const int Ho = deconv ? r.h_in : r.h_out, Wo = deconv ? r.w_in : r.w_out;
    c.TH = c.TW = 0;

    double best = -1;
    for (int WN = 1; WN <= 4; WN *= 2) {
        if (fwn && WN != fwn) continue;
        for (int NREP = 1; NREP <= 5; ++NREP) {
            if (fnrep && NREP != fnrep) continue;
            if (deconv && r.c2 % (16 * NREP)) continue;
            const int BN = WN * NREP;
            const int gy = (c.ntiles_n + BN - 1) / BN;
            const double n_eff = (double)c.ntiles_n / (gy * BN);
            if (n_eff < 0.74 && !fnrep) continue;
            const int BM = (4 / WN) * 80;
            for (int TW = std::min(Wo, BM); TW >= 1; --TW) {
                if (ftw && TW != ftw) continue;
                int TH = std::min(Ho, BM / TW);
                if (fth) { if (fth * TW > BM) continue; TH = fth; }
                if (TH < 1) continue;
                const int tiles = ((Ho + TH - 1) / TH) * ((Wo + TW - 1) / TW);
                const double m_eff = (double)Ho * Wo / ((double)tiles * BM);
                const int PH = conv0 ? TH : (TH - 1) * st + ks, PW = conv0 ? TW : (TW - 1) * st + ks;
                const size_t lds = conv_lds_bytes(ks, st, conv0 ? 1 : 0, TH, TW, WN, NREP);
                if (lds > ((fth || ftw) ? 160u : 80u) * 1024) continue;
                if (!conv_cfg_fits(ks, st, conv0 ? 1 : 0, TH, TW, WN, NREP)) continue;
                const double halo = conv0 ? (double)(4 * TH * TW) / ((2 * TH + 1) * (2 * TW + 1))
                                          : (double)(TH * TW * st * st) / (PH * PW);
                const double lds_traffic = 1.0 / NREP + 1.0 / 5;
                const double rowb = std::min(1.0, (double)TW * 64.0 / 1024.0);
                double score = m_eff * n_eff * (0.6 + 0.4 * halo) * (0.8 + 0.2 * rowb) / (0.35 + lds_traffic);
                if (lds > 64 * 1024) score *= 0.9;
                if (ks == 1 && WN >= 2) score *= 1.12;
                const double wgs = (double)tiles * gy * max_batch;
                if (wgs < 512) score *= 0.5 + 0.5 * wgs / 512;
                if (score > best) {
                    best = score;
                    c.TH = TH; c.TW = TW; c.WN = WN; c.NREP = NREP; c.lds = lds;
                }
            }
        }
    }
    if (c.TH) c.ntiles_n = (c.ntiles_n + c.NREP - 1) / c.NREP * c.NREP;
}

std::string Plan::build(const vti_desc& d) {
    desc = d;
    const Scale* sc = nullptr;
    for (const Scale& s : kScales) if (s.tag == d.scale) sc = &s;
    if (!sc) return "unknown scale (expected one of n,s,m,l,x)";
    if (d.nc < 1 || d.nm < 1 || d.reg_max < 1 || d.nm % 4 || d.nm > 64) return "bad nc/nm/reg_max";
    if (d.reg_max != 16) return "only reg_max=16 is supported";
    if (d.H < 32 || d.W < 32 || d.H % 32 || d.W % 32) return "H and W must be positive multiples of 32";
    if (d.max_batch < 1) return "max_batch must be >= 1";
    if (d.dtype != VTI_F16 && d.dtype != VTI_F32 && d.dtype != VTI_H2) return "dtype must be VTI_F16, VTI_F32 or VTI_H2";
    esize = d.dtype == VTI_F16 ? 2 : 4;

    auto ch = [&](int c) { return make_divisible(std::min(c, sc->maxc) * sc->width, 8); };
    auto rep = [&](int n) { return std::max(py_round(n * sc->depth), 1); };
    const int c0 = ch(64), c1 = ch(128), c2 = ch(256), c3 = ch(512), c4 = ch(1024);
    const int r0 = rep(3), r1 = rep(6), r2 = rep(6), r3 = rep(3), rn = rep(3);
    const int npr = ch(256);
    const int c_box = std::max(std::max(16, c2 / 4), 4 * d.reg_max);
    const int c_cls = std::max(c2, std::min(d.nc, 100));
    const int c_mc = std::max(c2 / 4, d.nm);
    for (int c : {c0, c1, c2, c3, c4, npr, c_box, c_cls, c_mc})
        if (c % 16) return "channel count not a multiple of 16 for this scale";

    Builder b(*this);
    std::vector<Op> g_p3, g_proto, g_head[3], g_p4, g_p5;
    b.cur = &g_p3;
    const int H = d.H, W = d.W;
    const int in_u8 = b.new_buf(3, H, W, EL_U8);
    const int B0 = b.new_buf(c0, H / 2, W / 2);
    const int B1 = b.new_buf(c1, H / 4, W / 4);
    const int B2 = b.new_buf(c1, H / 4, W / 4);
    const int B3 = b.new_buf(c2, H / 8, W / 8);
    const int CAT14 = b.new_buf(c3 + c2, H / 8, W / 8);
    const int B5 = b.new_buf(c3, H / 16, W / 16);
    const int CAT11 = b.new_buf(c4 + c3, H / 16, W / 16);
    const int B7 = b.new_buf(c4, H / 32, W / 32);
    const int B8 = b.new_buf(c4, H / 32, W / 32);
    const int SP = b.new_buf(2 * c4, H / 32, W / 32);
    const int CAT20 = b.new_buf(c3 + c4, H / 32, W / 32);
    const int CAT17 = b.new_buf(c2 + c3, H / 16, W / 16);
    const int P3 = b.new_buf(c2, H / 8, W / 8);
    const int P4 = b.new_buf(c3, H / 16, W / 16);
    const int P5 = b.new_buf(c4, H / 32, W / 32);

    b.conv("model.0", b.whole(in_u8), b.whole(B0), 3, 2, 0);
    b.conv("model.1", b.whole(B0), b.whole(B1), 3, 2, 0);
    b.c2f(2, b.whole(B1), b.whole(B2), r0, true);
    b.conv("model.3", b.whole(B2), b.whole(B3), 3, 2, 0);
    const View x4 = b.slice(CAT14, c3, c2);
    b.c2f(4, b.whole(B3), x4, r1, true);
    b.conv("model.5", x4, b.whole(B5), 3, 2, 0);
    const View x6 = b.slice(CAT11, c4, c3);
    b.c2f(6, b.whole(B5), x6, r2, true);
    b.conv("model.7", x6, b.whole(B7), 3, 2, 0);
    b.c2f(8, b.whole(B7), b.whole(B8), r3, true);
    const View x9 = b.slice(CAT20, c3, c4);
    b.conv("model.9.cv1", b.whole(B8), b.slice(SP, 0, c4 / 2), 1, 1, 0);
    { Op op; op.kind = OP_POOL; op.in = b.slice(SP, 0, c4 / 2); op.out = b.slice(SP, c4 / 2, 3 * (c4 / 2)); b.cur->push_back(op); }
    b.conv("model.9.cv2", b.whole(SP), x9, 1, 1, 0);
    b.up2(x9, b.slice(CAT11, 0, c4));
    const View x12 = b.slice(CAT17, c2, c3);
    b.c2f(12, b.whole(CAT11), x12, rn, false);
    b.up2(x12, b.slice(CAT14, 0, c3));
    b.c2f(15, b.whole(CAT14), b.whole(P3), rn, false);
    b.cur = &g_p4;
    b.conv("model.16", b.whole(P3), b.slice(CAT17, 0, c2), 3, 2, 0);
    b.c2f(18, b.whole(CAT17), b.whole(P4), rn, false);
    b.cur = &g_p5;
    b.conv("model.19", b.whole(P4), b.slice(CAT20, 0, c3), 3, 2, 0);
    b.c2f(21, b.whole(CAT20), b.whole(P5), rn, false);
    const int feat[3] = {P3, P4, P5};
    const int strides[3] = {8, 16, 32};
    num_anchors = 0;
    static const bool p3l = getenv("VTI_P3_LANES") && getenv("VTI_P3_LANES")[0] == '1';
    const int tower_lane[3][3] = {{2, p3l ? 8 : 2, p3l ? 9 : 2}, {3, 4, 5}, {6, 7, 0}};
    for (int l = 0; l < 3; ++l) {
        b.cur = &g_head[l];
        const Buf fb = bufs[feat[l]];
        Level lv; lv.C = fb.C; lv.H = fb.H; lv.W = fb.W; lv.stride = strides[l];
        const char* towers[3] = {"cv2", "cv3", "cv4"};
        const int cmid[3] = {c_box, c_cls, c_mc};
        const int cout[3] = {4 * d.reg_max, d.nc, d.nm};
        int outs[3];
        for (int t = 0; t < 3; ++t) {
            b.lane = tower_lane[l][t];
            const int t1 = b.new_buf(cmid[t], fb.H, fb.W), t2 = b.new_buf(cmid[t], fb.H, fb.W);
            outs[t] = b.new_buf(cout[t], fb.H, fb.W, EL_F32);
            char nm[64];
            snprintf(nm, sizeof nm, "model.22.%s.%d.0", towers[t], l);
            b.conv(nm, b.whole(feat[l]), b.whole(t1), 3, 1, 0);
            snprintf(nm, sizeof nm, "model.22.%s.%d.1", towers[t], l);
            b.conv(nm, b.whole(t1), b.whole(t2), 3, 1, 0);
            snprintf(nm, sizeof nm, "model.22.%s.%d.2", towers[t], l);
            b.conv(nm, b.whole(t2), b.whole(outs[t]), 1, 1, 1, true);
        }
        lv.box_buf = outs[0]; lv.cls_buf = outs[1]; lv.mc_buf = outs[2];
        levels.push_back(lv);
        num_anchors += fb.H * fb.W;
    }
    b.cur = &g_proto;
    b.lane = 1;
    {
        const int pc1 = b.new_buf(npr, H / 8, W / 8), pup = b.new_buf(npr, H / 4, W / 4);
        const bool proto_f32 = d.dtype == VTI_H2;
        const int pc2 = b.new_buf(npr, H / 4, W / 4), pout = b.new_buf(d.nm, H / 4, W / 4, proto_f32 ? EL_F32 : EL_T);
        b.conv("model.22.proto.cv1", b.whole(P3), b.whole(pc1), 3, 1, 0);
        b.conv("model.22.proto.upsample", b.whole(pc1), b.whole(pup), 2, 2, 2);
        b.conv("model.22.proto.cv2", b.whole(pup), b.whole(pc2), 3, 1, 0);
        b.conv("model.22.proto.cv3", b.whole(pc2), b.whole(pout), 1, 1, 0, proto_f32);
        proto_buf_c = pout;
    }
    {
        auto sync = [&](OpKind k, int lane) { Op op; op.kind = k; op.lane = lane; ops.push_back(op); };
        auto add = [&](const std::vector<Op>& g) { ops.insert(ops.end(), g.begin(), g.end()); };
        add(g_p3);
        sync(OP_FORK, 1); sync(OP_FORK, 2);
        if (p3l) { sync(OP_FORK, 8); sync(OP_FORK, 9); }
        add(g_proto); add(g_head[0]);
        add(g_p4);
        sync(OP_FORK, 3); sync(OP_FORK, 4); sync(OP_FORK, 5);
        add(g_head[1]);
        add(g_p5);
        sync(OP_FORK, 6); sync(OP_FORK, 7);
        add(g_head[2]);
        for (int l = 1; l <= (p3l ? 9 : 7); ++l) sync(OP_JOIN, l);
        Op op; op.kind = OP_DECODE; ops.push_back(op);
    }

    size_t off = 0;
    for (size_t i = 0; i < bufs.size(); ++i) {
        if ((int)i == in_u8 || (int)i == proto_buf_c) { bufs[i].off = 0; continue; }
        bufs[i].off = off;
        off += (bufs[i].bytes + 255) & ~(size_t)255;
    }
    ws_bytes = off;

    {
        const char* nf = getenv("VTI_NO_FUSE");
        for (size_t i = 0; !(nf && nf[0] == '1') && i + 1 < ops.size(); ++i) {
            Op& a = ops[i];
            const Op& b2 = ops[i + 1];
            if (a.kind != OP_CONV || b2.kind != OP_CONV || a.lane != b2.lane) continue;
            const ConvRow& ra = convs[a.conv];
            const ConvRow& rb = convs[b2.conv];
            if (!(ra.k == 3 && ra.s == 1 && ra.kind == 0 && rb.k == 1 && rb.s == 1 && rb.kind != 2)) continue;
            if (a.has_res || b2.has_res || a.out_f32) continue;
// ... 294 lines not shown
```

vision-textile-inspection_amd/csrc/vti_api.cpp:

```cpp
#include <algorithm>
#include <cmath>
#include <cstdio>
#include <cstdlib>
#include <cstring>
#include <new>

#include "vti_internal.h"
#include "rawframes_dev.h"

using namespace vti;

struct vti_ctx {
    Plan plan;
    std::string err;
    int device = -1;
    void* d_wpk = nullptr;
    float* d_bias = nullptr;
    std::vector<float> alpha;
    char* ws = nullptr;
    size_t ws_bytes = 0;
    size_t act_bytes = 0;
    const void* last_input = nullptr;
    void* last_proto = nullptr;
    hipStream_t side[kNumLanes] = {};
// ... 203 lines not shown
    if (!c || !frames || !out || H0 < 1 || W0 < 1 || B < 0) return fail(c, VTI_ERR_ARG, "vti_letterbox: bad argument");
    if (int32_t drc = check_device(c, "vti_letterbox")) return drc;
    VTI_HIP(c, launch_letterbox(frames, B, H0, W0, nullptr, out, c->plan.desc.H, c->plan.desc.W, (hipStream_t)stream),
            "letterbox kernel");
    return VTI_OK;
}

static const int32_t kFrameMaxSide = 16384;

int64_t vti_frame_table_bytes(int32_t B) {
    return B < 1 ? 0 : (int64_t)sizeof(FrameTableHeader) + (int64_t)B * (int64_t)sizeof(FrameRow);
}

static const char* frame_error(int32_t H, int32_t W, int32_t H0, int32_t W0, int64_t offset, int64_t total_bytes) {
    if (H0 < 1 || W0 < 1) return "H0 and W0 must be >= 1";
    if (H0 > kFrameMaxSide || W0 > kFrameMaxSide) return "H0 and W0 must be <= 16384";
    if (offset < 0 || (offset & 15)) return "byte_offset must be >= 0 and a multiple of 16";
    if (offset > total_bytes || 3 * (int64_t)H0 * W0 > total_bytes - offset) return "the frame runs past total_bytes";
    int nh, nw, top, left;
    letterbox_geom(H0, W0, H, W, nh, nw, top, left);
    if (nh < 1 || nw < 1) return "the resized frame would be below 1 px";
    if (top < 0 || left < 0 || top + nh > H || left + nw > W) return "the resized frame does not fit the canvas";
    return nullptr;
}

int32_t vti_pack_frames(vti_ctx* c, int32_t H, int32_t W, const int32_t* H0, const int32_t* W0, const int64_t* byte_offset, int32_t B,
                        int64_t total_bytes, void* host_table, size_t nbytes) {
    if (!H0 || !W0 || !byte_offset || !host_table || B < 1)
        return fail(c, VTI_ERR_ARG, "vti_pack_frames: null array or table, or B < 1");
    if (H < 32 || W < 32 || (H & 31) || (W & 31) || total_bytes < 0)
        return fail(c, VTI_ERR_ARG, "vti_pack_frames: the canvas H, W must be multiples of 32, total_bytes >= 0");
    if ((int64_t)nbytes < vti_frame_table_bytes(B))
        return fail(c, VTI_ERR_ARG, "vti_pack_frames: table smaller than vti_frame_table_bytes()");
    for (int32_t b = 0; b < B; ++b)
        if (const char* e = frame_error(H, W, H0[b], W0[b], byte_offset[b], total_bytes)) {
            char msg[200];
            snprintf(msg, sizeof msg, "vti_pack_frames: frame %d: %s", b, e);
            return fail(c, VTI_ERR_ARG, msg);
        }
    FrameTableHeader h;
    memset(&h, 0, sizeof h);
    h.magic = kFrameTableMagic; h.B = B; h.H = H; h.W = W; h.total_bytes = total_bytes;
    for (int32_t b = 0; b < B; ++b) {
        FrameRow r;
        frame_row_fill(H, W, H0[b], W0[b], byte_offset[b], r);
        h.max_H0 = std::max(h.max_H0, H0[b]); h.max_W0 = std::max(h.max_W0, W0[b]);
        memcpy((char*)host_table + sizeof h + (size_t)b * sizeof r, &r, sizeof r);
    }
    memcpy(host_table, &h, sizeof h);
    return VTI_OK;
}

int32_t vti_frame_table_info(const void* host_table, int32_t b, int32_t out_i32[8], double out_f64[5]) {
    if (!host_table || !out_i32) return VTI_ERR_ARG;
    FrameTableHeader h;
    memcpy(&h, host_table, sizeof h);
    if (h.magic != kFrameTableMagic || h.B < 1 || b < -1 || b >= h.B) return VTI_ERR_ARG;
    if (b < 0) {
        const int32_t v[8] = {h.B, h.H, h.W, h.max_H0, h.max_W0, 0, (int32_t)(h.total_bytes & 0xffffffff), (int32_t)(h.total_bytes >> 32)};
        memcpy(out_i32, v, sizeof v);
        return VTI_OK;
    }
    FrameRow r;
    memcpy(&r, (const char*)host_table + sizeof h + (size_t)b * sizeof r, sizeof r);
    const int32_t v[8] = {r.H0, r.W0, r.new_h, r.new_w, r.top, r.left, (int32_t)(r.offset & 0xffffffff), (int32_t)(r.offset >> 32)};
    memcpy(out_i32, v, sizeof v);
    if (out_f64) { out_f64[0] = r.scale_x; out_f64[1] = r.scale_y; out_f64[2] = r.gain; out_f64[3] = r.padx; out_f64[4] = r.pady; }
    return VTI_OK;
}

static const char* frame_table_problem(const vti_ctx* c, const void* host_table, int32_t B, FrameTableHeader& h, int32_t& frame) {
    frame = -1;
    memcpy(&h, host_table, sizeof h);
    if (h.magic != kFrameTableMagic) return "host_table is not a table of vti_pack_frames";
    if (h.B < 1 || (B >= 0 && h.B != B)) return "the frame table was packed for another B";
    if (h.H != c->plan.desc.H || h.W != c->plan.desc.W) return "the frame table was packed for another canvas (H x W)";
    for (int32_t b = 0; b < h.B; ++b) {
        FrameRow r;
        memcpy(&r, (const char*)host_table + sizeof h + (size_t)b * sizeof r, sizeof r);
        const char* e = frame_error(h.H, h.W, r.H0, r.W0, r.offset, h.total_bytes);
        if (!e && (r.H0 > h.max_H0 || r.W0 > h.max_W0)) e = "larger than the table's recorded maximum";
        if (e) { frame = b; return e; }
    }
    return nullptr;
}

static int32_t frames_check(const char* fn, vti_ctx* c, const void* host_table, const void* dev_table, int32_t B, FrameTableHeader& h) {
    char msg[200];
    auto bad = [&](const char* what) { snprintf(msg, sizeof msg, "%s: %s", fn, what); return fail(c, VTI_ERR_ARG, msg); };
    if (!c) return VTI_ERR_ARG;
    if (!host_table || !dev_table) return bad("null frame table (host copy or device copy)");
    if ((uintptr_t)dev_table & 15) return bad("the device frame table must be 16-byte aligned");
    int32_t frame;
    if (B < 1) {
        memcpy(&h, host_table, sizeof h);
        return bad(h.magic != kFrameTableMagic ? "host_table is not a table of vti_pack_frames" : "the frame table was packed for another B");
    }
    if (const char* e = frame_table_problem(c, host_table, B, h, frame)) {
        if (frame < 0) return bad(e);
        snprintf(msg, sizeof msg, "%s: frame %d of host_table: %s", fn, frame, e);
        return fail(c, VTI_ERR_ARG, msg);
    }
    return VTI_OK;
}

static const FrameRow* frame_rows(const void* dev_table) { return (const FrameRow*)((const char*)dev_table + sizeof(FrameTableHeader)); }

int32_t vti_letterbox_frames(vti_ctx* c, const uint8_t* frames, const void* host_table, const void* dev_table, int32_t B,
                             uint8_t* out, void* stream) {
    FrameTableHeader h;
    if (int32_t rc = frames_check("vti_letterbox_frames", c, host_table, dev_table, B, h)) return rc;
    if (!frames || !out) return fail(c, VTI_ERR_ARG, "vti_letterbox_frames: null frames or output");
    if (((uintptr_t)frames & 15) || ((uintptr_t)out & 3))
        return fail(c, VTI_ERR_ARG, "vti_letterbox_frames: dev_frames must be 16-byte aligned, dev_input 4-byte aligned");
    if (B > c->plan.desc.max_batch) return fail(c, VTI_ERR_ARG, "vti_letterbox_frames: B above max_batch");
    if (int32_t drc = check_device(c, "vti_letterbox_frames")) return drc;
    VTI_HIP(c, launch_letterbox(frames, B, 0, 0, frame_rows(dev_table), out, h.H, h.W, (hipStream_t)stream), "letterbox kernel");
    return VTI_OK;
}

static void* buf_ptr(vti_ctx* c, int buf, const void* input, void* proto) {
    if (buf == 0) return (void*)input;
    if (buf == c->plan.proto_buf_c) return proto;
    return c->ws + c->plan.bufs[buf].off;
}

static int stagger_units(int dtype) {
    static const int v = getenv("VTI_PK_STAGGER") ? std::max(0, std::min(255, atoi(getenv("VTI_PK_STAGGER")))) : -1;
    return v >= 0 ? v : (dtype == VTI_H2 ? 10 : 0);
}

static int pk_linear_map() {
    static const int v = getenv("VTI_PK_LINEAR_MAP") && getenv("VTI_PK_LINEAR_MAP")[0] == '1';
    return v;
}

static int scalar_store(int n, int ld, int coff) { return (n % 4 || ld % 4 || coff % 4) ? 1 : 0; }

static void fill_conv_params(int conv_elem_size, ConvParams& p, const ConvRow& r, const ConvCfg& g, int B, const void* in, int in_ld,
                             int in_coff, void* out, int out_ld, int out_coff, const void* res, int res_ld,
                             int res_coff, const void* wpk, const float* bias, bool out_f32, int swap_rb) {
    const bool deconv = r.kind == 2;
    memset(&p, 0, sizeof p);
    p.in = in; p.out = out; p.wpk = wpk; p.bias = bias;
    p.B = B; p.Hin = r.h_in; p.Win = r.w_in;
    p.Hout = deconv ? r.h_in : r.h_out; p.Wout = deconv ? r.w_in : r.w_out;
    p.Cin = r.c1; p.in_ld = in_ld; p.in_coff = in_coff;
    p.Cout = g.gemm_n; p.out_ld = out_ld; p.out_coff = out_coff;
    if (res) { p.res = res; p.res_ld = res_ld; p.res_coff = res_coff; p.has_res = 1; }
    p.TH = g.TH; p.TW = g.TW;
    p.tiles_y = (p.Hout + g.TH - 1) / g.TH; p.tiles_x = (p.Wout + g.TW - 1) / g.TW;
    p.WN = g.WN;
    p.nt = g.threads;
    p.pk_lin = pk_linear_map();
    p.act = r.kind == 0; p.out_f32 = out_f32 ? 1 : 0;
    p.deconv_c = deconv ? r.c2 : 0;
    p.swap_rb = swap_rb ? 1 : 0;
    p.nchunks = g.nchunks; p.ntiles_n = g.ntiles_n;
    p.scalar_store = scalar_store(g.gemm_n, out_ld, out_coff);
    const bool conv0 = r.c1 == 3;
    const int ks = deconv ? 1 : r.k, st = deconv ? 1 : r.s;
    const unsigned PW = conv0 ? (unsigned)g.TW : (unsigned)((g.TW - 1) * st + ks);
    p.pw_magic = (unsigned)((0x100000000ull + PW - 1) / PW);
    const unsigned RWD = ((unsigned)(2 * g.TW + 1) * 3 + 6) >> 2;
    p.rw_magic = (unsigned)((0x100000000ull + RWD - 1) / RWD);
    p.tw_magic = (unsigned)((0x100000000ull + (unsigned)g.TW - 1) / (unsigned)g.TW);
    p.wpk_bytes = (unsigned)packed_conv_bytes(r, conv0, g);
    if (g.pk == 2) {
        const size_t es = conv_elem_size;
        const size_t npx = (size_t)B * p.Hout * p.Wout;
        const size_t ib = npx * in_ld * es;
        const size_t ob = (deconv ? 4 * npx : npx) * out_ld * (out_f32 ? 4 : es);
        p.pk = (ib < 0x80000000ull && ob < 0x80000000ull && !res) ? 2 : 0;
        p.in_bytes = (unsigned)ib; p.out_bytes = (unsigned)ob; p.res_bytes = 0;
        p.pk_depth = g.pk_depth; p.pk_wstat = g.pk_wstat; p.pk_cps = g.pk_cps;
        p.pk_tiles = (int)((npx + (size_t)g.TH * 80 - 1) / ((size_t)g.TH * 80));
        p.pk_wgs = pk_grid(p.pk_tiles, g.pk_wgpc, g.ntiles_n / (g.WN * g.NREP), getenv("VTI_PK_MAX_WGS"));
        p.pk_xcd = p.pk_wgs >= 8 ? 1 : 0;
    } else if (g.pk) {
        const size_t es = conv_elem_size;
        const size_t ib = (size_t)B * r.h_in * r.w_in * in_ld * es, ob = (size_t)B * p.Hout * p.Wout * out_ld * (out_f32 ? 4 : es);
        const size_t rb = res ? (size_t)B * p.Hout * p.Wout * res_ld * es : 0;
        p.pk = (ib < 0x80000000ull && ob < 0x80000000ull && rb < 0x80000000ull) ? g.pk : 0;
        p.in_bytes = (unsigned)ib; p.out_bytes = (unsigned)ob; p.res_bytes = (unsigned)rb;
        p.pk_tiles = B * p.tiles_y * p.tiles_x;
        p.pk_depth = g.pk_depth; p.pk_wstat = g.pk_wstat;
        const int gy = g.ntiles_n / (g.WN * g.NREP);
        p.pk_wgs = pk_grid(p.pk_tiles, g.pk_wgpc, gy, getenv("VTI_PK_MAX_WGS"));
        p.pk_xcd = p.pk_wgs >= 8 ? 1 : 0;
        p.pk_stagger = ((g.pk == 1 || g.pk == 4) && p.pk_tiles >= std::max(1, 256 * g.pk_wgpc / gy) && p.pk_wgs >= 16) ? 1 : 0;
    }
}

static void fill_stage2(vti_ctx* c, ConvParams& p, const Op& op, const void* input, void* proto) {
    const Plan& P = c->plan;
    const ConvCfg& g = op.cfg;
    const Buf& o2 = P.bufs[op.out2.buf];
    p.w2 = (const char*)c->d_wpk + g.wpk_off2; p.bias2 = c->d_bias + g.bias_off2; p.alpha2 = c->alpha[op.fused];
    p.out2 = buf_ptr(c, op.out2.buf, input, proto);
    p.Cout2 = g.gemm_n2; p.ntiles2 = g.ntiles2; p.out2_ld = o2.C; p.out2_coff = op.out2.coff;
    p.act2 = P.convs[op.fused].kind == 0; p.out2_f32 = op.out2_f32 ? 1 : 0;
    p.scalar_store2 = scalar_store(g.gemm_n2, o2.C, op.out2.coff);
    p.nat2 = op.nat2;
    p.out2_bstride = P.convs[op.conv].h_out * P.convs[op.conv].w_out;
}

static int32_t forward_impl(vti_ctx* c, const uint8_t* input, int32_t B, int32_t swap_rb, float* pred, void* proto, float* best, void* stream);

int32_t vti_forward(vti_ctx* c, const uint8_t* input, int32_t B, int32_t swap_rb, float* pred, void* proto, void* stream) {
    return forward_impl(c, input, B, swap_rb, pred, proto, nullptr, stream);
}

int32_t vti_forward_scored(vti_ctx* c, const uint8_t* input, int32_t B, int32_t swap_rb, float* pred, void* proto, float* anchor_best,
                           void* stream) {
    if (!anchor_best) return fail(c, VTI_ERR_ARG, "vti_forward_scored: null pointer");
    return forward_impl(c, input, B, swap_rb, pred, proto, anchor_best, stream);
}

static int32_t forward_impl(vti_ctx* c, const uint8_t* input, int32_t B, int32_t swap_rb, float* pred, void* proto, float* best, void* stream) {
    int32_t rc = check_ready(c, B, "vti_forward");
    if (rc) return rc;
    if (!input || !pred || !proto) return fail(c, VTI_ERR_ARG, "vti_forward: null pointer");
    if (B == 0) return VTI_OK;
    const Plan& P = c->plan;
    hipStream_t main_st = (hipStream_t)stream;
    const int dt = P.desc.dtype;
    static const bool list_ops = getenv("VTI_LIST_OPS") != nullptr;
    if (list_ops) {
        int i = 0;
        for (const Op& op : P.ops) {
            if (op.kind == OP_FORK || op.kind == OP_JOIN) continue;
            const bool cv = op.kind == OP_CONV || op.kind == OP_CONV0;
            fprintf(stderr, "[op %2d] lane %d %s%s%s\n", i++, op.lane,
                    cv ? P.convs[op.conv].name.c_str() : op.kind == OP_POOL ? "sppf_pool" : op.kind == OP_UP2 ? "upsample2x" : "decode",
                    cv && op.fused_l1 >= 0 ? (" + " + P.convs[op.fused_l1].name).c_str() : cv && op.fold >= 0 ? (" (folded: " + P.convs[op.fold].name + ")").c_str() : cv && op.pair >= 0 ? (" + " + P.convs[op.pair].name + (op.tail >= 0 ? " + " + P.convs[op.tail].name : "")).c_str() : "",
                    cv && op.fused >= 0 ? (" + " + P.convs[op.fused].name).c_str() : "");
        }
    }
    for (const Op& op : P.ops) {
        hipStream_t st = (c->multi_stream && op.lane > 0) ? c->side[op.lane] : main_st;
        switch (op.kind) {
        case OP_FORK:
            if (c->multi_stream) {
                VTI_HIP(c, hipEventRecord(c->ev_fork[op.lane], main_st), "fork record");
                VTI_HIP(c, hipStreamWaitEvent(c->side[op.lane], c->ev_fork[op.lane], 0), "fork wait");
            }
            break;
        case OP_JOIN:
            if (c->multi_stream) {
                VTI_HIP(c, hipEventRecord(c->ev_join[op.lane], c->side[op.lane]), "join record");
                VTI_HIP(c, hipStreamWaitEvent(main_st, c->ev_join[op.lane], 0), "join wait");
            }
            break;
        case OP_CONV0:
        case OP_CONV: {
            const ConvRow& r = P.convs[op.conv];
            const ConvCfg& g = op.cfg;
            const Buf& ib = P.bufs[op.in.buf];
            const Buf& ob = P.bufs[op.out.buf];
            if (op.fused_l1 >= 0) {
                const ConvRow& r1 = P.convs[op.fused_l1];
                const Buf& o1 = P.bufs[op.out2.buf];
                ConvParams q;
                memset(&q, 0, sizeof q);
                q.in = input; q.B = B; q.Hin = r.h_in; q.Win = r.w_in; q.Hout = r1.h_out; q.Wout = r1.w_out;
                q.Cin = 16; q.Cout = r1.c2; q.ntiles_n = 2; q.act = 1; q.swap_rb = swap_rb ? 1 : 0;
                q.out = buf_ptr(c, op.out2.buf, input, proto); q.out_ld = o1.C; q.out_coff = op.out2.coff;
                q.wpk = (const char*)c->d_wpk + g.wpk_off2; q.bias = c->d_bias + g.bias_off2;
                q.w0 = (const char*)c->d_wpk + g.wpk_off; q.bias0 = c->d_bias + g.bias_off;
                q.alpha = c->alpha[op.fused_l1]; q.alpha0 = c->alpha[op.conv]; q.alpha2 = op.fused >= 0 ? c->alpha[op.fused] : 1.f;
                if (op.fused >= 0) {
                    q.out = nullptr;
                    q.w2 = (const char*)c->d_wpk + g.wpk_off3; q.bias2 = c->d_bias + g.bias_off3;
                    q.out2 = buf_ptr(c, op.out2.buf, input, proto);
                    q.Cout2 = g.gemm_n2; q.ntiles2 = g.ntiles2; q.out2_ld = o1.C; q.out2_coff = op.out2.coff;
                    q.act2 = 1; q.out2_bstride = r1.h_out * r1.w_out;
                    q.scalar_store2 = scalar_store(g.gemm_n2, o1.C, op.out2.coff);
                }
                stem_l1_tile(&q.TH, &q.TW);
                q.tiles_y = (q.Hout + q.TH - 1) / q.TH; q.tiles_x = (q.Wout + q.TW - 1) / q.TW; q.WN = 1;
                q.scalar_store = scalar_store(q.Cout, q.out_ld, q.out_coff);
#ifdef VTI_STAMPS
                if (const char* so = getenv("VTI_STAMP_OP"); so && r.name == so)
                    stamped_launch(q, (size_t)stem_l1_grid(dt, B * q.tiles_y * q.tiles_x), false, st,
                                   ("[stamps] op " + r.name + " + layer 1 (1: patch staged, 2: stem done, 3: layer-1 MFMAs done, 12: end)").c_str(),
                                   [&] { return launch_stem_l1(dt, q, st); });
#endif
                VTI_HIP(c, launch_stem_l1(dt, q, st), "stem + layer 1");
                break;
            }
            if (op.fold >= 0) {
                const ConvRow& ru = P.convs[op.fold];
                ConvParams q;
                memset(&q, 0, sizeof q);
                q.in = buf_ptr(c, op.in.buf, input, proto); q.B = B; q.Hin = ru.h_in; q.Win = ru.w_in; q.Hout = ru.h_in; q.Wout = ru.w_in;
                q.Cin = ru.c1; q.in_ld = ib.C; q.in_coff = op.in.coff; q.Cout = g.gemm_n; q.act = 1; q.fold = 1; q.pk_lin = pk_linear_map();
                q.TH = g.TH; q.TW = g.TW; q.tiles_y = (q.Hout + g.TH - 1) / g.TH; q.tiles_x = (q.Wout + g.TW - 1) / g.TW; q.WN = 4; q.nt = g.threads;
                q.nchunks = g.nchunks; q.ntiles_n = g.ntiles_n;
                q.pw_magic = (unsigned)((0x100000000ull + (unsigned)(g.TW + 2) - 1) / (unsigned)(g.TW + 2));
                q.tw_magic = (unsigned)((0x100000000ull + (unsigned)g.TW - 1) / (unsigned)g.TW);
                q.wpk = (const char*)c->d_wpk + g.wpk_off; q.bias = c->d_bias + g.bias_off; q.wpk_bytes = (unsigned)packed_fold_bytes(g);
                q.alpha = c->alpha[op.conv]; q.alpha0 = 1.f;
                fill_stage2(c, q, op, input, proto);
                if (g.pk) {
                    q.pk = 1; q.pk_depth = g.pk_depth; q.in_bytes = (unsigned)((size_t)B * q.Hin * q.Win * q.in_ld * P.esize);
                    q.pk_tiles = B * q.tiles_y * q.tiles_x;
// ... 1214 lines not shown
```

vision-textile-inspection_amd/csrc/vti_internal.h:

```cpp
#pragma once
#include <hip/hip_runtime.h>
#include <stddef.h>
#include <stdint.h>
#include <algorithm>
#include <cstdlib>
#include <string>
#include <vector>

#include "../../include/vti.h"
#include "jpeg_decode_dev.h"

namespace vti {

constexpr int kMaxDevices = 64;
inline int current_device_slot() { int d = 0; (void)hipGetDevice(&d); return (unsigned)d < (unsigned)kMaxDevices ? d : 0; }

template <auto K, typename... A>
hipError_t launch_lds(dim3 grid, dim3 block, size_t lds, hipStream_t st, const A&... args) {
    static size_t opted_dev[kMaxDevices] = {};
    size_t& opted = opted_dev[current_device_slot()];
    if (lds > 64 * 1024 && lds > opted) {
        hipError_t e = hipFuncSetAttribute((const void*)K, hipFuncAttributeMaxDynamicSharedMemorySize, (int)lds);
        if (e != hipSuccess) return e;
        opted = lds;
    }
    hipLaunchKernelGGL(K, grid, block, lds, st, args...);
    return hipGetLastError();
}

template <auto K>
int resident_per_cu(int threads, int fallback, int cap) {
    static int per_cu_dev[kMaxDevices] = {};
    int& per_cu = per_cu_dev[current_device_slot()];
    if (!per_cu) {
        int nb = 0;
        if (hipOccupancyMaxActiveBlocksPerMultiprocessor(&nb, (const void*)K, threads, 0) != hipSuccess || nb < 1) nb = fallback;
        per_cu = nb > cap ? cap : nb;
    }
    return per_cu;
}

inline int pk_grid(long tiles, int wgpc, int gy, const char* cap = nullptr) {
    long G = std::min<long>(tiles, std::max(1, 256 * wgpc / gy));
    if (cap) G = std::max<long>(1, std::min<long>(G, atoi(cap)));
    return (int)(G >= 8 ? G & ~7L : G);
}

enum ElemKind { EL_T = 0, EL_F32 = 1, EL_U8 = 2 };

struct Buf {
    int C, H, W;
    int elem;
    size_t off;
    size_t bytes;
};

struct View {
    int buf = -1, coff = 0, C = 0;
};

struct ConvRow {
    std::string name;
    int c1, c2, k, s, kind;
    int h_in, w_in, h_out, w_out;
    int64_t macs() const {
        const int64_t hw = (kind == 2) ? (int64_t)h_in * w_in : (int64_t)h_out * w_out;
        return hw * c1 * c2 * k * k;
    }
    int64_t fused_params() const { return (int64_t)c1 * c2 * k * k + c2; }
};

enum OpKind { OP_CONV0, OP_CONV, OP_POOL, OP_UP2, OP_DECODE, OP_FORK, OP_JOIN };
constexpr int kNumLanes = 10;

struct ConvCfg {
    int TH = 0, TW = 0;
    int WN = 1;
    int NREP = 1;
    int nchunks = 0;
    int ntiles_n = 0;
    int gemm_n = 0;
    size_t lds = 0;
    size_t wpk_off = 0;
    size_t bias_off = 0;
    int ntiles2 = 0, gemm_n2 = 0;
    size_t wpk_off2 = 0, bias_off2 = 0;
    size_t wpk_off3 = 0, bias_off3 = 0;
    int pk = 0, pk_wgpc = 1;
    int pk_depth = 2, pk_wstat = 0;
    int pk_cps = 1;
    int threads = 256;
};

struct Op {
    OpKind kind;
    int conv = -1;
    View in, out, res;
    bool has_res = false;
    bool out_f32 = false;
    int fused = -1;
    int tail = -1;
    int pair = -1;
    int fold = -1;
    int fused_l1 = -1;
    int pred_mode = 0, pred_cbase = 0, pred_a0 = 0;
    int dfl_stride = 0;
    int nat2 = 0;
    View out2;
    bool out2_f32 = false;
    View up_src; int up_C = 0;
    int lane = 0;
    ConvCfg cfg;
};

struct Level { int C, H, W, stride; int box_buf, cls_buf, mc_buf; };

struct Plan {
    vti_desc desc;
    int esize = 2;
    std::vector<ConvRow> convs;
    std::vector<View> conv_out;
    std::vector<Buf> bufs;
    std::vector<Op> ops;
    std::vector<Level> levels;
    int proto_buf_c = 0;
    View proto_src;
    int num_anchors = 0;
    bool pred_scatter = false;
    bool dfl_fused = false;
    size_t ws_bytes = 0;
    size_t wpk_bytes = 0, bias_floats = 0;
    int64_t macs = 0, fused_params = 0;
    std::string build(const vti_desc& d);
};

struct ConvParams {
    const void* in; void* out; const void* res; const void* wpk; const float* bias;
    int B, Hin, Win, Hout, Wout;
    int Cin, in_ld, in_coff;
    int Cout;
    int out_ld, out_coff, res_ld, res_coff;
    int TH, TW, tiles_y, tiles_x, WN;
    int act, out_f32, deconv_c, swap_rb, nchunks, ntiles_n, has_res, scalar_store;
    unsigned pw_magic, rw_magic, tw_magic;
    unsigned wpk_bytes;
    const void* w2; const float* bias2; void* out2;
    int Cout2, ntiles2, out2_ld, out2_coff, act2 , out2_f32, scalar_store2, nat2, out2_bstride;
    int nt;
    float* best;
    float dfl_stride;
    int pk, pk_tiles, pk_wgs, pk_xcd, pk_depth, pk_wstat, pk_lin ;
    int pk_cps;
    int pk_stagger;
    unsigned in_bytes, out_bytes, res_bytes, out2_bytes;
    const void* in2; int in2_ld, in2_coff, up_C; unsigned in2_bytes;
    int fold;
    const void* w0; const float* bias0;
    float alpha, alpha2, alpha0;
    unsigned long long* stamps;
};

hipError_t launch_conv(int dtype, int ks, int stride, int nrep, int mode, const ConvParams& p,
                       size_t lds_bytes, hipStream_t st);
bool conv_fusable(int nrep, int nrep2);
size_t conv_lds_bytes(int ks, int stride, int mode, int TH, int TW, int WN, int NREP);
bool conv_cfg_fits(int ks, int stride, int mode, int TH, int TW, int WN, int NREP, int threads = 256);
hipError_t launch_stem_l1(int dtype, const ConvParams& p, hipStream_t st);
size_t stem_l1_lds_bytes(int dtype);
void stem_l1_tile(int* th, int* tw);
int stem_l1_grid(int dtype, int ntiles);
void pack_stem_toeplitz(int dtype, const ConvRow& r0, const float* w, const float* b, uint8_t* dst_w, float* dst_b, float* alpha = nullptr);
size_t packed_stem_toeplitz_bytes(int dtype);
hipError_t launch_convfold(int dtype, const ConvParams& p, size_t lds_bytes, hipStream_t st);
size_t convfold_lds_bytes(int TH, int TW);
bool convfold_supported(int c_in, int c_mid, int c_out, int ntiles2);
void pack_conv_fold(int dtype, const ConvRow& rU, const ConvRow& rV, const ConvCfg& c, const float* wU, const float* bU,
                    const float* wV, const float* bV, uint8_t* dst_w, float* dst_b, float* alpha = nullptr);
size_t packed_fold_bytes(const ConvCfg& c);
hipError_t launch_conv_pk_fold(int dtype, const ConvParams& p, size_t lds_bytes, hipStream_t st);
size_t conv_pk_fold_lds_bytes(int nchunks, int depth);
int conv_pk_fold_depth(int nchunks);
void pack_conv_l1pairs(int dtype, const ConvRow& r1, const float* w, const float* b, uint8_t* dst_w, float* dst_b, float* alpha = nullptr);
size_t packed_l1pairs_bytes(int dtype);
hipError_t launch_conv_pk(int dtype, int nrep, const ConvParams& p, size_t lds_bytes, hipStream_t st);
size_t conv_pk_lds_bytes(int TH, int WN, int NREP, int nchunks);
size_t conv_pk_lds_bytes(int TH, int WN, int NREP, int nchunks, int depth, int wstat = 0);
int conv_pk_depth(int TH, int WN, int NREP, int nchunks, int wstat = 0);
hipError_t launch_conv_pk2(int dtype, int nrep, const ConvParams& p, size_t lds_bytes, hipStream_t st);
size_t conv_pk2_lds_bytes(int TH, int WN, int NREP, int nchunks, int depth, int wstat = 0);
bool conv_pk2_fits(int TH, int WN, int NREP, int nchunks, int wstat = 0);
bool conv_pk2_instantiated(int nrep, int wn);
int conv_pk2_depth(int TH, int WN, int NREP, int nchunks, int wstat = 0);
bool conv_pk_fits(int TH, int WN, int NREP, int nchunks, int wstat = 0);
bool conv_pk_instantiated(int nrep, int wn);
hipError_t launch_conv1_pk(int dtype, int nrep, const ConvParams& p, size_t lds_bytes, hipStream_t st);
size_t conv1_pk_lds_bytes(int nwm, int WN, int NREP, int nchunks, int depth, int wstat, int cps = 1);
bool conv1_pk_fits(int nwm, int WN, int NREP, int nchunks, int depth, int wstat, int cps = 1);
bool conv1_pk_instantiated(int nrep, int wn);
hipError_t launch_bneck_pk(int dtype, int nrep, const ConvParams& p, size_t lds_bytes, hipStream_t st);
size_t bneck_pk_lds_bytes(int TH, int NREP);
size_t bneck_pk_lds_bytes(int TH, int NREP, int depth);
int bneck_pk_depth(int TH, int NREP);
bool bneck_pk_fits(int TH, int NREP);

struct PoolParams { const void* in; void* out; int B, H, W, C, ld, in_coff, out_coff; };
hipError_t launch_sppf_pool(int dtype, const PoolParams& p, hipStream_t st);

struct Up2Params { const void* in; void* out; int B, H, W, C, in_ld, in_coff, out_ld, out_coff; };
hipError_t launch_upsample2x(int dtype, const Up2Params& p, hipStream_t st);

struct DecodeParams {
    const float* box[3]; const float* cls[3]; const float* mc[3];
    int H[3], W[3], stride[3], a0[3];
    int B, A, nc, nm, reg_max;
    float* pred;
};
hipError_t launch_decode(const DecodeParams& p, hipStream_t st);
hipError_t launch_box_decode(const DecodeParams& p, hipStream_t st);

hipError_t launch_debug_nchw(int elem_is_f32, const void* src, int B, int H, int W, int C, int ld, int coff,
                             float* dst, hipStream_t st);

struct FrameRow {
    long long offset;
    int H0, W0, new_h, new_w, top, left;
    double scale_x, scale_y;
    float gain, padx, pady;
    int pad;
};
static_assert(sizeof(FrameRow) == 64, "frame table rows are 64 bytes");
constexpr int kFrameTableMagic = 0x31544656;
struct FrameTableHeader {
    int magic, B, H, W, max_H0, max_W0;
    long long total_bytes;
    int pad[8];
};
static_assert(sizeof(FrameTableHeader) == 64, "the rows of a frame table stay 64-byte aligned");
void letterbox_geom(int H0, int W0, int H, int W, int& new_h, int& new_w, int& top, int& left);
void frame_row_fill(int H, int W, int H0, int W0, long long offset, FrameRow& r);

hipError_t launch_letterbox(const uint8_t* frames, int B, int H0, int W0, const FrameRow* table, uint8_t* out, int H, int W,
                            hipStream_t st);
size_t nms_workspace_bytes(int B, int A);
hipError_t launch_nms(const float* pred, const float* best, int B, int A, int nc, int nm, float conf, double iou, int max_det,
                      int agnostic, float* dets, int* counts, void* ws, hipStream_t st);
hipError_t launch_anchor_best(const float* pred, int B, int A, int nc, int nm, float* best, hipStream_t st);
float* nms_workspace_best(void* ws, int B, int A);
hipError_t launch_masks(int dtype, const float* dets, const int* counts, const void* proto, int B, int max_det,
                        int nm, int Hp, int Wp, int H, int W, int mode, int packing, uint8_t* masks,
                        int capacity, int* offsets, void* ws, hipStream_t st);
size_t masks_workspace_bytes(int capacity, int H, int W);
int native_mask_layout(int Hp, int Wp, int H0, int W0, int packing, int out[6]);
hipError_t launch_masks_native(int dtype, const float* dets, const float* xyxy, const int* counts, const void* proto, int B, int max_det,
                               int Hp, int Wp, int H0, int W0, int mode, int packing, uint8_t* masks, int capacity, int* offsets,
                               void* ws, hipStream_t st);
long long native_frames_bytes(const void* host_table, int Hp, int Wp, int max_det, long long* tiles);
size_t masks_native_frames_workspace_bytes(int B);
hipError_t launch_masks_native_frames(int dtype, const float* dets, const float* xyxy, const int* counts, const void* proto,
                                      const FrameRow* rows, int B, int max_det, int Hp, int Wp, int mode, uint8_t* masks,
                                      long long capacity_bytes, int* offsets, long long* bases, void* ws, hipStream_t st);
hipError_t launch_scale_boxes(const float* dets, const int* counts, int B, int max_det, int nm, int H, int W,
                              int H0, int W0, const FrameRow* table, float* xyxy, hipStream_t st);
hipError_t launch_mask_to_frame(const uint8_t* masks, int n, int H, int W, int H0, int W0, uint8_t* bitmaps,
                                int* nonzero, hipStream_t st);
hipError_t launch_union_envelope(const uint8_t* bitmaps, const int* select, int nsel, int H0, int W0,
                                 uint8_t* uni, int* envelope, hipStream_t st);
hipError_t launch_mask_stats(const uint8_t* bitmaps, int n, int H0, int W0, long long* stats, hipStream_t st);

hipError_t launch_mask_stats_bits(const uint8_t* bits, int n, const int* n_live, int H, int W, int H0, int W0, long long* stats,
                                  hipStream_t st);
hipError_t launch_envelope_bits(const uint8_t* bits, const int* offsets, const float* dets, int B, int max_det, int nm,
                                int capacity, int cls, int H, int W, int H0, int W0, int* envelope, hipStream_t st);
hipError_t launch_pixels_to_world(const double* uv, int n, const double* K, const double* dist, const double* R,
                                  const double* t, double* xyz, int* valid, hipStream_t st);
hipError_t launch_kmeans1d2(const double* values, const int* counts, int B, int max_n, int max_iters, int* labels,
                            double* centers, hipStream_t st);
void measure_scratch_layout(int B, int capacity, int W0, size_t off[3], size_t& total);
size_t measure_camera_row_bytes();
void measure_pack_camera(const vti_measure_params& p, void* row);
hipError_t launch_measure(const vti_measure_params* p, const void* table, int n_cams, const int* cam_of_frame, const uint8_t* masks,
                          int native, const float* dets, const float* xyxy, const int* counts, const int* offsets, int B, int max_det,
                          int nm, int capacity, int H, int W, int H0, int W0, const FrameRow* frames, void* scratch, double* frame_f64,
                          int* frame_i32, double* stitch_f64, int* stitch_i32, hipStream_t st, const long long* bases = nullptr,
                          long long capacity_bytes = 0);

hipError_t launch_measure_checker(const vti_checker_params& p, const uint8_t* masks, int native, const float* dets, const float* xyxy,
                                  const int* counts, const int* offsets, int B, int max_det, int nm, int capacity, int H, int W, int H0,
                                  int W0, void* scratch, double* frame_f64, int* frame_i32, double* stitch_f64, int* stitch_i32,
                                  hipStream_t st);

#define VTI_POLY_WORKGROUPS 128
struct PolyLayout {
    int WW;
    bool in_lds;
    size_t img_bytes, off_runs, off_rows, off_img, area_bytes, total;
};
void mask_polygons_layout(int H, int W, int row_bytes, PolyLayout& L);
hipError_t launch_mask_polygons(const uint8_t* masks, int n, const int* n_live, int H, int W, int row_bytes, double gain,
                                double padx, double pady, int H0, int W0, int strategy, void* scratch, int* offsets, float* points,
                                long long max_points, hipStream_t st);

struct AnnotateLayout {
    int WW;
    bool in_lds;
    size_t off_recs, off_meta, off_env, off_cont, off_union, off_areas, area_bytes, off_runs, off_rows, total;
};
void annotate_layout(int n_sel, int max_det, int H0, int W0, int max_points, AnnotateLayout& L);
struct AnnotateFrames { const FrameRow* rows_in; const FrameRow* rows_out; bool any_lds, any_global; long long max_px; };
hipError_t launch_annotate(const uint8_t* frames, int B, int H0, int W0, const void* cameras, int n_cams, const int* cam_of_frame,
                           const uint8_t* masks, int native, const float* dets, const float* xyxy, const int* counts,
                           const int* offsets, int max_det, int nm, int capacity, int H, int W, const int* frame_i32,
                           const double* stitch_f64, const int* stitch_i32, const int* select, int n_sel, int max_points, uint8_t* out,
                           int* status, void* scratch, hipStream_t st, const AnnotateFrames* fr = nullptr);

struct OverlayLayout {
    int WW, groups;
    bool in_lds;
    size_t off_meta, off_cont, off_planes, off_areas, plane_words, area_bytes, off_runs, off_rows, off_img, total;
};
void overlay_layout(int n_sel, int max_det, int H0, int W0, int Hm, int Wm, int max_points, OverlayLayout& L);
struct OverlayFrames {
    const FrameRow* rows_in; const FrameRow* rows_out; const long long* bases; long long capacity_bytes, max_slot_words;
    bool any_lds, any_global; long long max_px;
};
hipError_t launch_overlay(const uint8_t* frames, int B, int H0, int W0, const uint8_t* masks, int native, const float* dets,
                          const float* xyxy, const int* counts, const int* offsets, int max_det, int nm, int capacity, int H, int W,
                          const int* plates, const uint8_t* palette, int n_colours, float alpha, float beta, const int* select,
                          int n_sel, int mode, const uint8_t* annotated, int max_points, uint8_t* out, int* status, void* scratch,
                          hipStream_t st, const OverlayFrames* fr = nullptr);

struct JpegLayout {
    int mr, mc;
    long long nblk;
    long long stream_bytes;
    long long NC;
    long long max_file;
    size_t off_fbits, off_fsize, off_coef, off_bitpos, off_stream, off_chunk, total;
};
bool encode_jpeg_layout(long long n, int H0, int W0, JpegLayout& L);
void encode_jpeg_header(int H0, int W0, int quality, uint8_t out[624]);
hipError_t launch_encode_jpeg(const uint8_t* frames, int n, int H0, int W0, int rgb, int quality, void* scratch, long long* offsets,
                              uint8_t* out, long long max_bytes, hipStream_t st);
struct JpegFramesLayout {
    int n;
    long long n_mcu, n_chunk;
    long long max_bytes;
    size_t off_pm, off_pc, off_fbits, off_fsize, off_coef, off_bitpos, off_stream, off_chunk, total;
};
bool encode_jpeg_frames_layout(const void* host_table, JpegFramesLayout& L);
hipError_t launch_encode_jpeg_frames(const uint8_t* frames, const void* host_table, const FrameRow* rows, int rgb, int quality,
                                     void* scratch, long long* offsets, uint8_t* out, long long max_bytes, hipStream_t st);
// ... 24 lines not shown
```

Measured before the change: 15990.

## Keep 1x1 conv weights in registers instead of LDS for persistent and tiled kernels

Adds a register-resident weight path for 1x1 convolutions. In the generic conv kernel each wave loads its own weight fragments straight into VGPRs rather than staging them through LDS. In the persistent conv1_pk kernel all chunk weights are loaded once per workgroup into registers, pre-split into hi/lo halves for f16x2, and the chunk count is compiled in. The planner's cost model now scores the register variant alongside the existing ones. This removes LDS weight traffic and barriers-bound copies but raises register pressure and adds many template instantiations.

```diff
diff --git a/vision-textile-inspection_amd/csrc/conv.hip b/vision-textile-inspection_amd/csrc/conv.hip
--- a/vision-textile-inspection_amd/csrc/conv.hip
+++ b/vision-textile-inspection_amd/csrc/conv.hip
@@ -10,17 +10,21 @@
 
 size_t stem_lds_bytes(int TH, int TW);
 
-size_t conv_lds_bytes(int ks, int stride, int mode, int TH, int TW, int WN, int NREP) {
+bool conv_wreg_ok(int ks, int stride, int mode, int WN, int NREP, int threads) {
+    return mode == 0 && ks == 1 && stride == 1 && threads == 256 && WN == 4 && NREP <= 4;
+}
+
+size_t conv_lds_bytes(int ks, int stride, int mode, int TH, int TW, int WN, int NREP, int wreg) {
     if (mode == 1) return stem_lds_bytes(TH, TW);
     const int npix = patch_dim(TH, ks, stride, mode) * patch_dim(TW, ks, stride, mode);
     const size_t plane = (size_t)((npix + 15) & ~15) * 16;
     const int taps = mode == 1 ? 1 : ks * ks;
     size_t raw = 0;
     if (mode == 1) raw = (((size_t)(2 * TH + 1) * (2 * TW + 1) * 3) + 15) & ~(size_t)15;
-    return 4 * plane + (size_t)WN * NREP * taps * 1024 + raw;
-}
-
-template <typename T, int KS, int S, int NREP, int WN, int NREP2 = 0, int NT = 256>
+    return 4 * plane + (wreg ? 0 : (size_t)WN * NREP * taps * 1024) + raw;
+}
+
+template <typename T, int KS, int S, int NREP, int WN, int NREP2 = 0, int NT = 256, bool WREG = false>
 __global__ __launch_bounds__(NT, NT == 512 ? 1 : 2) void conv_kernel(const ConvParams p) {
     using vec = typename Tr<T>::vec;
     constexpr int VEC = Tr<T>::VEC, KC = Tr<T>::KC;
@@ -29,6 +33,7 @@
     constexpr int PP = NT / 4;
     constexpr int AR = NT == 512 ? 6 : (S == 2 ? 12 : 8);
     constexpr int BR = (NTB * TAPS * 64 + NT - 1) / NT;
+    static_assert(!WREG || (KS == 1 && WN == NT / 64 && NREP2 == 0 && BR == NREP && NREP < 5), "WREG: one consumer wave per fragment");
     constexpr unsigned OOB = 0xFFFFFFFFu;
     extern __shared__ __attribute__((aligned(16))) char smem[];
 
@@ -92,8 +97,10 @@
     auto loadB = [&](int c, vec (&rbs)[BR]) {
         const unsigned sB = (unsigned)(((size_t)c * p.ntiles_n + nt0) * (TAPS * 1024));
 #pragma unroll
-        for (int u = 0; u < BR; ++u)
-            if (tid + u * NT < NTB * TAPS * 64) rbs[u] = buf_load16<vec>(rsB, (unsigned)(tid + u * NT) * 16u, sB);
+        for (int u = 0; u < BR; ++u) {
+            if constexpr (WREG) rbs[u] = buf_load16<vec>(rsB, (unsigned)((wn * NREP + u) * 64 + lane) * 16u, sB);
+            else if (tid + u * NT < NTB * TAPS * 64) rbs[u] = buf_load16<vec>(rsB, (unsigned)(tid + u * NT) * 16u, sB);
+        }
     };
     auto issue = [&](int c, vec (&ras)[AR], vec (&rbs)[BR]) {
         const bool qok = c < cvalid;
@@ -108,9 +115,11 @@
 #pragma unroll
         for (int u = 0; u < AR; ++u)
             if (pix0 + PP * u < npix) *(vec*)(smA + ldsA0 + u * (PP * 16)) = ras[u];
-#pragma unroll
-        for (int u = 0; u < BR; ++u)
-            if (tid + u * NT < NTB * TAPS * 64) *(vec*)(smB + (tid + u * NT) * 16) = rbs[u];
+        if constexpr (!WREG) {
+#pragma unroll
+            for (int u = 0; u < BR; ++u)
+                if (tid + u * NT < NTB * TAPS * 64) *(vec*)(smB + (tid + u * NT) * 16) = rbs[u];
+        }
     };
     auto chunk = [&](int c, auto set_c) {
         constexpr int SET = decltype(set_c)::value;
@@ -119,13 +128,17 @@
         if (c < 2) VTI_STAMP(3 + 5 * c);
         __syncthreads();
         if (c < 2) VTI_STAMP(4 + 5 * c);
+        constexpr int WD = NREP >= 5 ? 1 : 2;
+        vec wq[WD][NREP];
+        if constexpr (WREG) {
+#pragma unroll
+            for (int n = 0; n < NREP; ++n) wq[0][n] = rb[SET][n];
+        }
         if (c + PD < p.nchunks) issue(c + PD, ra[SET], rb[SET]);
         {
             constexpr int NSTEP = TAPS * MREP;
             constexpr int XD = NREP >= 5 ? 2 : 3;
-            constexpr int WD = NREP >= 5 ? 1 : 2;
             vec xq[XD];
-            vec wq[WD][NREP];
             auto ldx = [&](int s_) -> vec {
                 const int tp = s_ / MREP, mm = s_ % MREP;
                 const int toff = ((tp / KS) * PW + (tp % KS)) * 16;
@@ -140,7 +153,7 @@
                 auto ldw1 = [&](int tp, int n) -> vec { return *(const vec*)(smB + ((wn * NREP + n) * TAPS + tp) * 1024 + lane * 16); };
                 h2_taps<NREP, MREP, TAPS, 3>(acc, ldx, ldw1);
             } else {
-            ldw(0, wq[0]);
+            if constexpr (!WREG) ldw(0, wq[0]);
             xq[0] = ldx(0);
             if (XD > 2 && NSTEP > 1) xq[1] = ldx(1);
 #pragma unroll
@@ -705,6 +718,7 @@
 
 using ConvTile3 = Combos<Ints<1, 1>, Ints<2, 1>, Ints<3, 1>, Ints<4, 1>, Ints<5, 1>, Ints<1, 2>, Ints<2, 2>, Ints<1, 4>>;
 using ConvTile1 = decltype(concat(ConvTile3{}, Combos<Ints<3, 2>, Ints<4, 2>, Ints<5, 2>, Ints<2, 4>, Ints<3, 4>, Ints<4, 4>, Ints<5, 4>>{}));
+using ConvTile1W = Combos<Ints<1, 4>, Ints<2, 4>, Ints<3, 4>, Ints<4, 4>>;
 using StemNrep = Combos<Ints<1>, Ints<2>, Ints<3>, Ints<4>, Ints<5>>;
 
 bool conv_cfg_fits(int ks, int stride, int mode, int TH, int TW, int WN, int NREP, int threads) {
@@ -720,6 +734,12 @@
 
 template <typename T, int KS, int S>
 static hipError_t launch_ks(int nrep, const ConvParams& p, dim3 grid, size_t lds, hipStream_t st) {
+    if constexpr (KS == 1) {
+        if (p.wreg)
+            return combo_dispatch(ConvTile1W{}, [&](auto c) {
+                return launch_lds<conv_kernel<T, 1, 1, decltype(c)::v[0], 4, 0, 256, true>>(grid, dim3(256), lds, st, p);
+            }, nrep, p.WN);
+    }
     return combo_dispatch(std::conditional_t<KS == 1, ConvTile1, ConvTile3>{}, [&](auto c) {
         using C = decltype(c);
         return launch_lds<conv_kernel<T, KS, S, C::v[0], C::v[1]>>(grid, dim3(256), lds, st, p);
@@ -758,6 +778,8 @@
     dim3 grid((unsigned)(p.B * p.tiles_y * p.tiles_x), (unsigned)((p.ntiles_n + NTB - 1) / NTB));
     if (grid.x == 0) return hipSuccess;
     const int nwaves = p.nt == 512 ? 8 : 4;
+    if (p.wreg && !conv_wreg_ok(ks, stride, mode, p.WN, nrep, p.nt)) return hipErrorInvalidValue;
+    lds_bytes = std::max(lds_bytes, conv_lds_bytes(ks, stride, mode, p.TH, p.TW, p.WN, nrep, p.wreg));
     if ((p.nt != 256 && p.nt != 512) || (p.nt == 512 && p.ntiles2 == 0)) return hipErrorInvalidValue;
     if (p.TH * p.TW > (nwaves / p.WN) * MREP * 16 || (p.WN != 1 && p.WN != 2 && p.WN != 4)) return hipErrorInvalidValue;
     return with_conv_type(dtype, [&](auto t) { return launch_t<typename decltype(t)::type>(ks, stride, nrep, mode, p, grid, lds_bytes, st); });
diff --git a/vision-textile-inspection_amd/csrc/conv_pk.hip b/vision-textile-inspection_amd/csrc/conv_pk.hip
--- a/vision-textile-inspection_amd/csrc/conv_pk.hip
+++ b/vision-textile-inspection_amd/csrc/conv_pk.hip
@@ -19,6 +19,15 @@
 bool conv_pk_instantiated(int nrep, int wn) { return combo_has(ConvPkS1{}, nrep, wn); }
 bool conv_pk2_instantiated(int nrep, int wn) { return combo_has(ConvPkS2{}, nrep, wn); }
 bool conv1_pk_instantiated(int nrep, int wn) { return combo_has(Conv1Pk{}, nrep, wn); }
+using Conv1PkWH2 = Combos<Ints<2, 2, 4>, Ints<2, 2, 6>, Ints<2, 2, 8>, Ints<2, 2, 12>, Ints<2, 2, 16>,
+                          Ints<2, 4, 4>, Ints<2, 4, 6>, Ints<2, 4, 8>, Ints<2, 4, 12>, Ints<2, 4, 16>>;
+using Conv1PkWF16 = Combos<Ints<2, 2, 2>, Ints<2, 2, 3>, Ints<2, 2, 4>, Ints<2, 2, 6>, Ints<2, 2, 8>,
+                           Ints<2, 4, 2>, Ints<2, 4, 3>, Ints<2, 4, 4>, Ints<2, 4, 6>, Ints<2, 4, 8>, Ints<4, 1, 2>>;
+using Conv1PkWF32 = Combos<>;
+template <typename T> using Conv1PkW = std::conditional_t<Tr<T>::H2, Conv1PkWH2, std::conditional_t<Tr<T>::F32, Conv1PkWF32, Conv1PkWF16>>;
+bool conv1_pk_wreg_instantiated(int dtype, int nrep, int wn, int nchunks) {
+    return dtype == VTI_H2 ? combo_has(Conv1PkWH2{}, nrep, wn, nchunks) : dtype == VTI_F16 ? combo_has(Conv1PkWF16{}, nrep, wn, nchunks) : false;
+}
 
 static size_t pk_stage_bytes(int TH, int S) { return S == 2 ? (size_t)(2 * TH + 1) * 2 * PK_PWP * 64 : (size_t)(TH + 2) * PK_PWP * 64; }
 size_t conv_pk2_lds_bytes(int TH, int WN, int NREP, int nchunks, int depth, int wstat) {
@@ -408,10 +417,16 @@
 size_t conv1_pk_lds_bytes(int nwm, int WN, int NREP, int nchunks, int depth, int wstat, int cps) {
     const size_t stage = (size_t)nwm * 80 * 64 * cps;
     const size_t wch = (size_t)WN * NREP * 1024;
-    return (size_t)depth * stage + (wstat ? (size_t)nchunks * wch : (size_t)depth * wch * cps) + 1024  + (size_t)WN * NREP * 64;
-}
-
-template <typename T, int NREP, int WN, int CPS>
+    const size_t wbytes = wstat == 2 ? 0 : wstat ? (size_t)nchunks * wch : (size_t)depth * wch * cps;
+    return (size_t)depth * stage + wbytes + 1024  + (size_t)WN * NREP * 64;
+}
+
+template <typename V> __device__ __forceinline__ void reg_touch(V& v) {
+    if constexpr (std::is_same<V, h2x4>::value) asm volatile("" : "+v"(v.u));
+    else asm volatile("" : "+v"(v));
+}
+
+template <typename T, int NREP, int WN, int CPS, int NCH = 0>
 __global__ __launch_bounds__(512) void conv1_pk(const ConvParams p) {
     using vec = typename Tr<T>::vec;
     constexpr int VEC = Tr<T>::VEC, KC = Tr<T>::KC, ES = (int)sizeof(T);
@@ -432,7 +447,7 @@
     const int stage_bytes = img_bytes * CPS;
     const int npieces = tile_px / 16;
     const int wbuf_off = D * stage_bytes;
-    const int dummy_off = wbuf_off + (p.pk_wstat ? p.nchunks : D * CPS) * WCH;
+    const int dummy_off = wbuf_off + (NCH > 0 ? 0 : p.pk_wstat ? p.nchunks : D * CPS) * WCH;
     const int spt = (p.nchunks + CPS - 1) / CPS;
     const int bias_off = dummy_off + 1024;
     const unsigned lds0 = (unsigned)(size_t)(__attribute__((address_space(3))) char*)smem;
@@ -462,7 +477,7 @@
         const __amdgpu_buffer_rsrc_t rsA = __builtin_amdgcn_make_buffer_rsrc((void*)p.in, 0, (int)p.in_bytes, 0x00020000);
         const __amdgpu_buffer_rsrc_t rsB = __builtin_amdgcn_make_buffer_rsrc((void*)p.wpk, 0, (int)p.wpk_bytes, 0x00020000);
         const int ppl = (npieces + nld - 1) / nld;
-        const int wpl = p.pk_wstat ? 0 : (NTB + nld - 1) / nld;
+        const int wpl = (NCH > 0 || p.pk_wstat) ? 0 : (NTB + nld - 1) / nld;
         const int per_step = CPS * (ppl + wpl);
         const __amdgpu_buffer_rsrc_t rsA2 = __builtin_amdgcn_make_buffer_rsrc((void*)p.in2, 0, (int)p.in2_bytes, 0x00020000);
         unsigned vo1[PK1_MAXP], vo2[PK1_MAXP];
@@ -515,7 +530,7 @@
                 }
             }
         };
-        if (p.pk_wstat) {
+        if (NCH == 0 && p.pk_wstat) {
             for (int f = lw; f < p.nchunks * NTB; f += nld) {
                 const int c = f / NTB, n = f - c * NTB;
                 dma16(rsB, (unsigned)lane * 16u, (unsigned)(((size_t)c * p.ntiles_n + nt0 + n) * 1024), lds0 + wbuf_off + f * 1024);
@@ -544,15 +559,101 @@
                           (sizeof(T) != 2 || NREP % 2 || (p.Cout & 7) == 0);
     const int crun = (nt0 + wn * NREP) * 16 + (lane >> 4) * 4 * NREP;
     int s = 0;
+    constexpr int NCHR = NCH > 0 ? NCH : 1;
+    constexpr bool PREP = Tr<T>::H2 && NCH > 0 && NCH * NREP <= 16;
+    [[maybe_unused]] vec wr[PREP ? 1 : NCHR][NREP];
+    [[maybe_unused]] u32x4 whi[PREP ? NCHR : 1][NREP], wlo[PREP ? NCHR : 1][NREP];
+    if constexpr (NCH > 0) {
+        const __amdgpu_buffer_rsrc_t rsW = __builtin_amdgcn_make_buffer_rsrc((void*)p.wpk, 0, (int)p.wpk_bytes, 0x00020000);
+        vec wld[NCH][NREP];
+        const unsigned wv0 = (unsigned)(nt0 + wn * NREP) * 1024u + (unsigned)lane * 16u;
+#pragma unroll
+        for (int c = 0; c < NCH; ++c)
+#pragma unroll
+            for (int n = 0; n < NREP; ++n) wld[c][n] = buf_load16<vec>(rsW, wv0 + (unsigned)(c * p.ntiles_n + n) * 1024u, 0u);
+#pragma unroll
+        for (int c = 0; c < NCH; ++c)
+#pragma unroll
+            for (int n = 0; n < NREP; ++n) {
+                if constexpr (PREP) {
+#pragma unroll
+                    for (int i = 0; i < 4; ++i) {
+                        whi[c][n][i] = __builtin_amdgcn_perm(wld[c][n].u[i], wld[c][n].u[i], 0x01000100u);
+                        wlo[c][n][i] = wld[c][n].u[i] >> 16;
+                    }
+                    reg_touch(whi[c][n]); reg_touch(wlo[c][n]);
+                } else {
+                    wr[c][n] = wld[c][n];
+                    reg_touch(wr[c][n]);
+                }
+            }
+    }
+    VTI_STAMP(0);
     for (int ti = 0; ti < ntiles_mine; ++ti) {
         f32x4 acc[MREP][NREP];
 #pragma unroll
         for (int m = 0; m < MREP; ++m)
 #pragma unroll
             for (int n = 0; n < NREP; ++n) acc[m][n] = (f32x4){0.f, 0.f, 0.f, 0.f};
+        if constexpr (NCH > 0) {
+            constexpr int SPT = (NCH + CPS - 1) / CPS;
+#pragma unroll
+            for (int cs = 0; cs < SPT; ++cs, ++s) {
+                if (s == 2) VTI_STAMP(1);
+                __builtin_amdgcn_s_barrier();
+                asm volatile("" ::: "memory");
+                if (s == 2) VTI_STAMP(2);
+                const char* sx = smem + (s % D) * stage_bytes;
+                const int ncc = NCH - cs * CPS < CPS ? NCH - cs * CPS : CPS;
+                vec x[MREP];
+#pragma unroll
+                for (int m = 0; m < MREP; ++m) x[m] = *(const vec*)(sx + xa[m]);
+#pragma unroll
+                for (int cc = 0; cc < CPS; ++cc) {
+                    if (cc < ncc) {
+                    const int c = cs * CPS + cc;
+                    [[maybe_unused]] const char* sxn = sx + (cc + 1) * img_bytes;
+                    [[maybe_unused]] unsigned sel_h = 0x01000100u, sh_l = 16u;
+                    if constexpr (Tr<T>::H2 && !PREP) asm volatile("" : "+s"(sel_h), "+s"(sh_l));
+                    if constexpr (Tr<T>::H2) {
+#pragma unroll
+                        for (int n = 0; n < NREP; ++n) {
+                            u32x4 wh_, wl_;
+                            if constexpr (PREP) { wh_ = whi[c][n]; wl_ = wlo[c][n]; }
+                            else {
+#pragma unroll
+                                for (int i = 0; i < 4; ++i) { wh_[i] = __builtin_amdgcn_perm(wr[c][n].u[i], wr[c][n].u[i], sel_h); wl_[i] = wr[c][n].u[i] >> sh_l; }
+                            }
+                            if constexpr (PREP) __builtin_amdgcn_sched_barrier(0);
+                            if (cc == 0 && n == 0 && s == 2) VTI_STAMP(3);
+#pragma unroll
+                            for (int j = 0; j < 2 * MREP; ++j) {
+                                const int m = j >> 1;
+                                acc[m][n] = __builtin_amdgcn_mfma_f32_16x16x32_f16(__builtin_bit_cast(half8, (j & 1) ? wl_ : wh_),
+                                                                                   __builtin_bit_cast(half8, x[m].u), acc[m][n], 0, 0, 0);
+                                if (n == NREP - 1 && (j & 1) && cc + 1 < ncc) x[m] = *(const vec*)(sxn + xa[m]);
+                            }
+                            if constexpr (PREP) __builtin_amdgcn_sched_barrier(0);
+                        }
+                    } else {
+                        if (cc == 0 && s == 2) VTI_STAMP(3);
+#pragma unroll
+                        for (int m = 0; m < MREP; ++m) {
+#pragma unroll
+                            for (int n = 0; n < NREP; ++n) acc[m][n] = mma(wr[c][n], x[m], acc[m][n]);
+                            if (cc + 1 < ncc) x[m] = *(const vec*)(sxn + xa[m]);
+                        }
+                    }
+                    }
+                }
+                if (s == 2) VTI_STAMP(4);
+            }
+        } else
         for (int cs = 0; cs < spt; ++cs, ++s) {
+            if (s == 2) VTI_STAMP(1);
             __builtin_amdgcn_s_barrier();
             asm volatile("" ::: "memory");
+            if (s == 2) VTI_STAMP(2);
             const int slot = s % D;
             const int ncc = min(CPS, p.nchunks - cs * CPS);
             if constexpr (Tr<T>::H2) {
@@ -581,6 +682,7 @@
                         u32x4 wnext = wraw[nxt];
                         if (u + 2 < nu) wraw[cur] = *(const u32x4*)wptr(u + 2);
                         __builtin_amdgcn_sched_barrier(0);
+                        if (u == 0 && s == 2) VTI_STAMP(3);
 #pragma unroll
                         for (int j = 0; j < 2 * MREP; ++j) {
                             const int m = j >> 1;
@@ -610,6 +712,7 @@
                         vec x[MREP];
 #pragma unroll
                         for (int m = 0; m < MREP; ++m) x[m] = *(const vec*)(sx + xa[m]);
+                        if (cc == 0 && s == 2) VTI_STAMP(3);
 #pragma unroll
                         for (int m = 0; m < MREP; ++m)
 #pragma unroll
@@ -617,6 +720,7 @@
                     }
                 }
             }
+            if (s == 2) VTI_STAMP(4);
         }
         const int pix0 = (t + ti * tstride) * tile_px + wm * 80;
         if (fast_epi) {
@@ -679,6 +783,7 @@
             conv_epilogue<T, NREP>(p, acc, pvalid, opy, opx, bfr, nt0, wn, lane);
         }
     }
+    VTI_STAMP(12);
 }
 
 bool conv1_pk_fits(int nwm, int WN, int NREP, int nchunks, int depth, int wstat, int cps) {
@@ -694,6 +799,7 @@
 hipError_t launch_conv1_pk(int dtype, int nrep, const ConvParams& p, size_t lds_bytes, hipStream_t st) {
     const int NTB = p.WN * nrep;
     if (!conv1_pk_fits(p.TH, p.WN, nrep, p.nchunks, p.pk_depth, p.pk_wstat, p.pk_cps)) return hipErrorInvalidValue;
+    if (lds_bytes < conv1_pk_lds_bytes(p.TH, p.WN, nrep, p.nchunks, p.pk_depth, p.pk_wstat, p.pk_cps)) return hipErrorInvalidValue;
     if (p.ntiles_n % NTB || p.pk_wgs < 1 || (p.pk_xcd && p.pk_wgs % 8) || p.has_res) return hipErrorInvalidValue;
     if ((size_t)p.in_bytes >= 0x80000000u || (size_t)p.out_bytes >= 0x80000000u) return hipErrorInvalidValue;
     if (p.pk_tiles == 0) return hipSuccess;
@@ -703,6 +809,13 @@
         using T = typename decltype(t)::type;
         constexpr int CPS = sizeof(T) == 2 ? 1 : 2;
         if (p.pk_cps != CPS) return hipErrorInvalidValue;
+        if (p.pk_wstat == 2) {
+            if (p.deconv_c) return hipErrorInvalidValue;
+            return combo_dispatch(Conv1PkW<T>{}, [&](auto c) {
+                using C = decltype(c);
+                return launch_lds<conv1_pk<T, C::v[0], C::v[1], CPS, C::v[2]>>(grid, dim3(threads), lds_bytes, st, p);
+            }, nrep, p.WN, p.nchunks);
+        }
         return combo_dispatch(Conv1Pk{}, [&](auto c) {
             using C = decltype(c);
             return launch_lds<conv1_pk<T, C::v[0], C::v[1], CPS>>(grid, dim3(threads), lds_bytes, st, p);
diff --git a/vision-textile-inspection_amd/csrc/plan.cpp b/vision-textile-inspection_amd/csrc/plan.cpp
--- a/vision-textile-inspection_amd/csrc/plan.cpp
+++ b/vision-textile-inspection_amd/csrc/plan.cpp
@@ -208,7 +208,13 @@
     return found;
 }
 
-static bool choose_pk1_cfg(int esize, const ConvRow& r, int max_batch, ConvCfg& c, int fth, int fwn, int fnrep) {
+static bool conv1_wreg_enabled() {
+    const char* e = getenv("VTI_CONV1_WREG");
+    return !(e && e[0] == '0');
+}
+
+static bool choose_pk1_cfg(int dtype, const ConvRow& r, int max_batch, ConvCfg& c, int fth, int fwn, int fnrep) {
+    const int esize = dtype == VTI_F16 ? 2 : 4;
     const int cps = esize == 2 ? 1 : 2;
     const char* no = getenv("VTI_NO_PK1");
     if (no && no[0] == '1') return false;
@@ -235,10 +241,13 @@
                 const int ncomp = nwm * WN;
                 if (ncomp > 4) continue;
                 static const size_t wstat_max = getenv("VTI_PK1_WSTAT_KB") ? (size_t)atoi(getenv("VTI_PK1_WSTAT_KB")) * 1024 : 96 * 1024;
-                const int wstat = (size_t)c.nchunks * NTB * 1024 <= wstat_max ? 1 : 0;
+                const int wstat_lds = (size_t)c.nchunks * NTB * 1024 <= wstat_max ? 1 : 0;
+                const bool wreg_ok = conv1_wreg_enabled() && !deconv && conv1_pk_wreg_instantiated(dtype, NREP, WN, c.nchunks);
+                for (int wreg = 0; wreg <= (wreg_ok ? 1 : 0); ++wreg) {
+                const int wstat = wreg ? 2 : wstat_lds;
                 static const bool no_w2 = getenv("VTI_PK1_NO_WGPC2") && getenv("VTI_PK1_NO_WGPC2")[0] == '1';
                 static const bool force_w2 = getenv("VTI_PK1_FORCE_WGPC2") && getenv("VTI_PK1_FORCE_WGPC2")[0] == '1';
-                for (int wgpc = (esize == 4 && force_w2) ? 2 : 1; wgpc <= ((esize == 4 && !no_w2) ? 2 : 1); ++wgpc) {
+                for (int wgpc = (esize == 4 && force_w2 && !wreg) ? 2 : 1; wgpc <= ((esize == 4 && !no_w2 && !wreg) ? 2 : 1); ++wgpc) {
                     int depth = 0;
                     for (int dd = 8; dd >= 2; --dd)
                         if (conv1_pk_fits(nwm, WN, NREP, c.nchunks, dd, wstat, cps) &&
@@ -247,8 +256,8 @@
                     const long NT = (total_px + nwm * 80 - 1) / (nwm * 80);
                     const long G = pk_grid(NT, wgpc, gy);
                     const long rounds = (NT + G - 1) / G;
-                    const double solo = esize == 4 ? ((ncomp * wgpc > 4) ? 1.1 : 1.45) : 1.0;
-                    const double step_cyc = 5.0 * NREP * 16 * solo * (esize == 4 ? 2.0 : 1.0) + 250.0 / cps;
+                    const double solo = esize == 4 ? ((ncomp * wgpc > 4 || wreg) ? 1.1 : 1.45) : 1.0;
+                    const double step_cyc = 5.0 * NREP * 16 * solo * (esize == 4 ? 2.0 : 1.0) + (wreg ? 120.0 : 250.0) / cps;
                     const double t_comp = rounds * (c.nchunks * step_cyc + 1100.0 * NREP) * ((ncomp * wgpc + 3) / 4) / 1.9e9;
                     const double bytes = (double)total_px * ((double)gy * r.c1 + (double)c.gemm_n) * esize +
                                          (wstat ? 0.0 : (double)NT * gy * c.nchunks * NTB * 1024 * 0.25);
@@ -260,7 +269,9 @@
                         best = cost; found = true;
                         c.TH = nwm; c.TW = 80; c.WN = WN; c.NREP = NREP; c.pk = 2; c.pk_wgpc = wgpc; c.pk_depth = depth; c.pk_wstat = wstat; c.pk_cps = cps;
                         c.lds = conv1_pk_lds_bytes(nwm, WN, NREP, c.nchunks, depth, wstat, cps);
+                        c.wreg = wreg;
                     }
+                }
                 }
             }
         }
@@ -278,7 +289,8 @@
     c.ntiles_n = (c.gemm_n + 15) / 16;
     c.nchunks = conv0 ? (32 / KC) : (r.c1 + KC - 1) / KC;
     c.pk = 0;
-    if (allow_pk && !conv0 && (!ftw || ftw == 80) && (!fth || fth <= 4) && choose_pk1_cfg(f16 ? 2 : 4, r, max_batch, c, fth, fwn, fnrep)) return;
+    c.wreg = 0;
+    if (allow_pk && !conv0 && (!ftw || ftw == 80) && (!fth || fth <= 4) && choose_pk1_cfg(dtype, r, max_batch, c, fth, fwn, fnrep)) return;
     c.pk_wstat = 0;
     if (allow_pk && !conv0 && (!ftw || ftw == 20) && (!fth || fth % 4 == 0) && choose_pk_cfg(dtype, r, max_batch, c, fth, fwn, fnrep)) {
         return;
@@ -307,7 +319,8 @@
                 const int tiles = ((Ho + TH - 1) / TH) * ((Wo + TW - 1) / TW);
                 const double m_eff = (double)Ho * Wo / ((double)tiles * BM);
                 const int PH = conv0 ? TH : (TH - 1) * st + ks, PW = conv0 ? TW : (TW - 1) * st + ks;
-                const size_t lds = conv_lds_bytes(ks, st, conv0 ? 1 : 0, TH, TW, WN, NREP);
+                const int wreg = conv1_wreg_enabled() && conv_wreg_ok(ks, st, conv0 ? 1 : 0, WN, NREP) ? 1 : 0;
+                const size_t lds = conv_lds_bytes(ks, st, conv0 ? 1 : 0, TH, TW, WN, NREP, wreg);
                 if (lds > ((fth || ftw) ? 160u : 80u) * 1024) continue;
                 if (!conv_cfg_fits(ks, st, conv0 ? 1 : 0, TH, TW, WN, NREP)) continue;
                 const double halo = conv0 ? (double)(4 * TH * TW) / ((2 * TH + 1) * (2 * TW + 1))
@@ -321,7 +334,7 @@
                 if (wgs < 512) score *= 0.5 + 0.5 * wgs / 512;
                 if (score > best) {
                     best = score;
-                    c.TH = TH; c.TW = TW; c.WN = WN; c.NREP = NREP; c.lds = lds;
+                    c.TH = TH; c.TW = TW; c.WN = WN; c.NREP = NREP; c.lds = lds; c.wreg = wreg;
                 }
             }
         }
diff --git a/vision-textile-inspection_amd/csrc/vti_api.cpp b/vision-textile-inspection_amd/csrc/vti_api.cpp
--- a/vision-textile-inspection_amd/csrc/vti_api.cpp
+++ b/vision-textile-inspection_amd/csrc/vti_api.cpp
@@ -379,6 +379,7 @@
     p.tiles_y = (p.Hout + g.TH - 1) / g.TH; p.tiles_x = (p.Wout + g.TW - 1) / g.TW;
     p.WN = g.WN;
     p.nt = g.threads;
+    p.wreg = g.pk ? 0 : g.wreg;
     p.pk_lin = pk_linear_map();
     p.act = r.kind == 0; p.out_f32 = out_f32 ? 1 : 0;
     p.deconv_c = deconv ? r.c2 : 0;
diff --git a/vision-textile-inspection_amd/csrc/vti_internal.h b/vision-textile-inspection_amd/csrc/vti_internal.h
--- a/vision-textile-inspection_amd/csrc/vti_internal.h
+++ b/vision-textile-inspection_amd/csrc/vti_internal.h
@@ -90,6 +90,7 @@
     int pk_depth = 2, pk_wstat = 0;
     int pk_cps = 1;
     int threads = 256;
+    int wreg = 0;
 };
 
 struct Op {
@@ -147,6 +148,7 @@
     const void* w2; const float* bias2; void* out2;
     int Cout2, ntiles2, out2_ld, out2_coff, act2 , out2_f32, scalar_store2, nat2, out2_bstride;
     int nt;
+    int wreg;
     float* best;
     float dfl_stride;
     int pk, pk_tiles, pk_wgs, pk_xcd, pk_depth, pk_wstat, pk_lin ;
@@ -163,7 +165,8 @@
 hipError_t launch_conv(int dtype, int ks, int stride, int nrep, int mode, const ConvParams& p,
                        size_t lds_bytes, hipStream_t st);
 bool conv_fusable(int nrep, int nrep2);
-size_t conv_lds_bytes(int ks, int stride, int mode, int TH, int TW, int WN, int NREP);
+size_t conv_lds_bytes(int ks, int stride, int mode, int TH, int TW, int WN, int NREP, int wreg = 0);
+bool conv_wreg_ok(int ks, int stride, int mode, int WN, int NREP, int threads = 256);
 bool conv_cfg_fits(int ks, int stride, int mode, int TH, int TW, int WN, int NREP, int threads = 256);
 hipError_t launch_stem_l1(int dtype, const ConvParams& p, hipStream_t st);
 size_t stem_l1_lds_bytes(int dtype);
@@ -197,6 +200,7 @@
 size_t conv1_pk_lds_bytes(int nwm, int WN, int NREP, int nchunks, int depth, int wstat, int cps = 1);
 bool conv1_pk_fits(int nwm, int WN, int NREP, int nchunks, int depth, int wstat, int cps = 1);
 bool conv1_pk_instantiated(int nrep, int wn);
+bool conv1_pk_wreg_instantiated(int dtype, int nrep, int wn, int nchunks);
 hipError_t launch_bneck_pk(int dtype, int nrep, const ConvParams& p, size_t lds_bytes, hipStream_t st);
 size_t bneck_pk_lds_bytes(int TH, int NREP);
 size_t bneck_pk_lds_bytes(int TH, int NREP, int depth);
```

Result: faster. 16240 (median of 6 runs) (+1.5%).
